# maxrossi91/moni-align

Measured on AMD Instinct MI355X. Metric: aligned reads/s (whole node), 150 bp SE, mouse-chr19-scale x12-haplotype index, higher is better.
Workload: dtype u64/int32

## Files before the change

include/moni_hip.h:

```cpp
#ifndef MONI_HIP_H
#define MONI_HIP_H

#include <stddef.h>
#include <stdint.h>

#ifdef __cplusplus
extern "C" {
#endif

#define MONI_OK 0
#define MONI_EINVAL (-22)
#define MONI_ENOMEM (-12)
#define MONI_EIO (-5)
#define MONI_ENODEV (-19)
#define MONI_ERANGE (-34)

typedef struct moni_index moni_index_t;
typedef struct moni_ctx moni_ctx_t;

typedef struct {
    uint64_t n;
    uint64_t r;
    uint64_t w;
    uint64_t n_seq;
// ... 46 lines not shown
    uint32_t n_cigar;
    uint32_t cigar_off;
} moni_dp_result_t;

typedef struct {
    uint64_t q_off, t_off;
    int32_t qlen, tlen;
    int32_t flag;
    int32_t reserved;
} moni_dp_task_t;

typedef struct {
    int8_t m;
    int8_t mat[25];
    int8_t q, e;
    int32_t w, zdrop, end_bonus;
} moni_dp_params_t;

int moni_index_create(const moni_flat_index_t *flat, int device, moni_index_t **out);
int moni_index_load(const char *path, int device, moni_index_t **out);
void moni_index_destroy(moni_index_t *idx);
uint64_t moni_index_n(const moni_index_t *idx);
uint64_t moni_index_r(const moni_index_t *idx);
uint64_t moni_index_device_bytes(const moni_index_t *idx);
int moni_index_text(const moni_index_t *idx, uint8_t *out, uint64_t cap);

int moni_ctx_create(moni_index_t *idx, moni_ctx_t **out);
void moni_ctx_destroy(moni_ctx_t *ctx);
int moni_reads_upload(moni_ctx_t *ctx, const moni_read_batch_t *batch);
int moni_reads_swap(moni_ctx_t *ctx, uint32_t slot);

int moni_ms_run(moni_ctx_t *ctx);
int moni_ms_query_batch(moni_ctx_t *ctx, const moni_read_batch_t *batch, uint64_t *pointers);

int moni_ms_lengths_batch(moni_ctx_t *ctx, const moni_read_batch_t *batch, uint64_t *pointers, uint64_t *lengths);

typedef struct { uint32_t seg_len;
                 uint32_t overlap;
                 uint32_t reserved[2]; } moni_mslong_params_t;
typedef struct { uint64_t patterns, bases, segments, flagged, chain_runs;
                 uint64_t steps_spec, steps_chain, jumps;
                 double t_walk, t_len, t_chain, t_total;
               } moni_mslong_stats_t;
void moni_mslong_params_default(moni_mslong_params_t *p);
int  moni_ms_long_batch(moni_ctx_t *ctx, const moni_read_batch_t *batch, const moni_mslong_params_t *prm,
                        uint64_t *pointers, uint64_t *lengths, moni_mslong_stats_t *stats);

int moni_seed_run(moni_ctx_t *ctx, const moni_seed_params_t *prm);
int moni_seed_counts(moni_ctx_t *ctx, uint64_t *n_mems, uint64_t *n_occs);
int moni_seed_fetch(moni_ctx_t *ctx, moni_mem_t *mems, uint64_t *occs, uint64_t *read_mem_off);
int moni_seed_batch(moni_ctx_t *ctx, const moni_read_batch_t *batch, const moni_seed_params_t *prm,
                    moni_mem_t **mems, uint64_t *n_mems, uint64_t **occs, uint64_t *n_occs, uint64_t **read_mem_off);
void moni_free(void *p);

int moni_phi_lcp_batch(moni_ctx_t *ctx, const uint64_t *pos, uint64_t n, int inverse, uint64_t *out_pos, uint64_t *out_lcp);

int moni_extz_batch(moni_ctx_t *ctx, const moni_dp_params_t *prm, const uint8_t *qseq, uint64_t qseq_len,
                    const uint8_t *tseq, uint64_t tseq_len, const moni_dp_task_t *tasks, uint64_t n_tasks,
                    moni_dp_result_t *results, uint32_t *cigar_pool, uint64_t cigar_pool_cap, uint64_t *cigar_pool_used);

typedef struct {
    uint32_t min_len, ext_len, check_k, region_dist;
    uint32_t filter_seeds, n_seeds_thr, filter_freq, left_mem_check;
    double freq_thr;
    int8_t smatch, smismatch, gapo, gapo2, gape, gape2;
    int32_t end_bonus, w, zdrop;
    int64_t max_dist_x, max_dist_y, max_iter, max_pred, min_chain_score, min_chain_length;
    uint32_t host_threads;
    uint32_t reserved;
} moni_align_params_t;

typedef struct {
    uint64_t reads, aligned, dp_tasks, dp_cells, dp_rounds;
    double t_seed, t_chain, t_dp, t_host;
    double t_dp_kernel;
    uint64_t handed_back;
    uint64_t dp_reused, dp_cells_reused;
    uint64_t kernel_fallback;
    uint64_t dp_ref_bytes;
    double t_k_chain, t_k_dp, t_k_select, t_k_finish;
    uint64_t handover_why[12];
    uint64_t dp_cells_cut;
    uint64_t dp_slots;
} moni_align_stats_t;

void moni_align_params_default(moni_align_params_t *p);
int moni_align_batch(moni_ctx_t *ctx, const moni_read_batch_t *batch, const uint8_t *names, const uint64_t *name_off,
                     const uint8_t *quals, const moni_align_params_t *prm, char **sam, uint64_t *sam_len,
                     moni_align_stats_t *stats);
int moni_align_run(moni_ctx_t *ctx, const uint8_t *names, const uint64_t *name_off, const uint8_t *quals,
                   const moni_align_params_t *prm, char **sam, uint64_t *sam_len, moni_align_stats_t *stats);
int moni_align_stream(moni_ctx_t *ctx, const moni_read_batch_t *batch, const uint8_t *names, const uint64_t *name_off,
                      const uint8_t *quals, const moni_align_params_t *prm, char **sam, uint64_t *sam_len,
                      moni_align_stats_t *stats);
int moni_align_csv_batch(moni_ctx_t *ctx, const moni_read_batch_t *batch, const uint8_t *names, const uint64_t *name_off,
                         const uint8_t *quals, const moni_align_params_t *prm, char **sam, uint64_t *sam_len,
                         char **csv, uint64_t *csv_len, moni_align_stats_t *stats);
int moni_report_mems_batch(moni_ctx_t *ctx, const moni_read_batch_t *batch, const uint8_t *names, const uint64_t *name_off,
                           const uint8_t *quals, const moni_align_params_t *prm, char **sam, uint64_t *sam_len);
typedef struct {
    uint32_t filter_dir, find_orphan;
    double dir_thr;
    uint64_t ins_learning_n;
    uint64_t ins_learning_score_gap_threshold;
    uint32_t secondary_chains, reserved;
} moni_pe_params_t;
typedef struct {
    double mean, std_dev, variance, sample_variance, m2;
    uint64_t count;
    uint32_t complete, reserved;
} moni_pe_model_t;
void moni_pe_params_default(moni_pe_params_t *p);
int moni_pe_learn_batch(moni_ctx_t *ctx, const moni_read_batch_t *batch, const moni_align_params_t *prm,
                        const moni_pe_params_t *pe, moni_pe_model_t *model);
int moni_pe_align_batch(moni_ctx_t *ctx, const moni_read_batch_t *batch, const uint8_t *names, const uint64_t *name_off,
                        const uint8_t *quals, const moni_align_params_t *prm, const moni_pe_params_t *pe,
                        const moni_pe_model_t *model, char **sam, uint64_t *sam_len, moni_align_stats_t *stats);
int moni_pe_align_stream(moni_ctx_t *ctx, const moni_read_batch_t *batch, const uint8_t *names, const uint64_t *name_off,
                        const uint8_t *quals, const moni_align_params_t *prm, const moni_pe_params_t *pe,
                        const moni_pe_model_t *model, char **sam, uint64_t *sam_len, moni_align_stats_t *stats);
int moni_pe_align_run(moni_ctx_t *ctx, const uint8_t *names, const uint64_t *name_off, const uint8_t *quals, const moni_align_params_t *prm,
                      const moni_pe_params_t *pe, const moni_pe_model_t *model, char **sam, uint64_t *sam_len, moni_align_stats_t *stats);
int moni_pe_align_csv_batch(moni_ctx_t *ctx, const moni_read_batch_t *batch, const uint8_t *names, const uint64_t *name_off,
                            const uint8_t *quals, const moni_align_params_t *prm, const moni_pe_params_t *pe,
                            const moni_pe_model_t *model, char **sam, uint64_t *sam_len, char **csv, uint64_t *csv_len,
                            moni_align_stats_t *stats);
int moni_pe_report_mems_batch(moni_ctx_t *ctx, const moni_read_batch_t *batch, const uint8_t *names, const uint64_t *name_off,
                              const uint8_t *quals, const moni_align_params_t *prm, const moni_pe_params_t *pe, char **sam, uint64_t *sam_len);
typedef struct {
    uint32_t min_len, ext_len;
    int8_t smatch, smismatch, gapo, gape;
    int32_t end_bonus, w, zdrop;
    uint32_t reserved;
} moni_extend_params_t;
typedef struct {
    uint64_t reads, extended, records;
    uint64_t dp_tasks, dp_cells;
    double t_kernel;
} moni_extend_stats_t;
void moni_extend_params_default(moni_extend_params_t *p);
int moni_extend_batch(moni_ctx_t *ctx, const moni_read_batch_t *batch, const uint8_t *names, const uint64_t *name_off, const uint8_t *quals,
                      const moni_extend_params_t *prm, char **sam, uint64_t *sam_len, moni_extend_stats_t *stats);
int moni_extend_run(moni_ctx_t *ctx, const uint8_t *names, const uint64_t *name_off, const uint8_t *quals, const moni_extend_params_t *prm,
                    char **sam, uint64_t *sam_len, moni_extend_stats_t *stats);
int moni_sam_header(const moni_index_t *idx, char **sam, uint64_t *sam_len);

int moni_pml_batch(moni_ctx_t *ctx, const moni_read_batch_t *batch, uint32_t thr,
                   uint32_t *lengths, uint32_t *read_max, uint32_t *read_hits);
int moni_pml_run(moni_ctx_t *ctx, uint32_t thr);
int moni_pml_fetch(moni_ctx_t *ctx, uint32_t *lengths, uint32_t *read_max, uint32_t *read_hits);
int moni_pml_sizes(moni_ctx_t *ctx, uint64_t *n_reads, uint64_t *total_len);

#define MONI_SCREEN_BINS 32
#define MONI_SCREEN_PRESENT 1u
#define MONI_SCREEN_STRAND1 2u
#define MONI_SCREEN_SHORT 4u
typedef struct { uint32_t window;
                 uint32_t min_win;
                 uint32_t ks_num, ks_den;
                 uint32_t strands;
                 uint32_t reserved[3]; } moni_screen_params_t;
typedef struct { uint32_t n_win, n_pos[2], d_max[2], max_pml[2], flags; } moni_screen_res_t;
void moni_screen_params_default(moni_screen_params_t *p);
int moni_screen_run(moni_ctx_t *ctx, const moni_screen_params_t *prm);
int moni_screen_sizes(moni_ctx_t *ctx, uint64_t *n_reads);
int moni_screen_fetch(moni_ctx_t *ctx, moni_screen_res_t *res);
// ... 82 lines not shown
```

moni_align_amd/capi.py:

```python
from __future__ import annotations

import ctypes as C
import os
import subprocess
from typing import Dict, Optional

import numpy as np

os.environ.setdefault("GPU_MAX_HW_QUEUES", "16")

HERE = os.path.dirname(os.path.abspath(__file__))
CSRC = os.path.join(HERE, "csrc")
LIB_PATH = os.environ.get("MONI_HIP_LIB") or os.path.join(CSRC, "libmoni_hip.so")

EXPORTS = [
    "moni_version", "moni_index_create", "moni_index_load", "moni_index_destroy", "moni_index_n", "moni_index_r",
    "moni_index_device_bytes", "moni_index_text", "moni_ctx_create", "moni_ctx_destroy", "moni_reads_upload", "moni_reads_swap", "moni_ms_run",
    "moni_ms_query_batch", "moni_seed_run", "moni_seed_counts", "moni_seed_fetch", "moni_seed_batch", "moni_free",
    "moni_phi_lcp_batch", "moni_extz_batch", "moni_last_kernel_ms", "moni_last_counters", "moni_seed_occ_stats",
    "moni_seed_prefilter", "moni_seed_prefilter_stats",
    "moni_align_params_default", "moni_align_batch", "moni_align_csv_batch", "moni_align_run", "moni_align_stream", "moni_sam_header",
    "moni_ldx_info", "moni_ldx_rewrite", "moni_ldx_lift_batch", "moni_ldx_write",
    "moni_ms_file_info", "moni_ms_file_read", "moni_ms_file_write", "moni_index_load_reference", "moni_ms_lengths_batch", "moni_report_mems_batch",
    "moni_pe_params_default", "moni_pe_learn_batch", "moni_pe_align_batch", "moni_pe_align_stream", "moni_pe_align_run", "moni_pe_align_csv_batch", "moni_pe_report_mems_batch",
    "moni_extend_params_default", "moni_extend_batch", "moni_extend_run",
    "moni_pml_batch", "moni_pml_run", "moni_pml_fetch", "moni_pml_sizes",
    "moni_screen_params_default", "moni_screen_run", "moni_screen_sizes", "moni_screen_fetch", "moni_screen_batch",
    "moni_locate_params_default", "moni_locate_run", "moni_locate_sizes", "moni_locate_fetch", "moni_locate_batch",
    "moni_seqcount_params_default", "moni_seqcount_run", "moni_seqcount_sizes", "moni_seqcount_fetch", "moni_seqcount_batch",
    "moni_loci_params_default", "moni_loci_run", "moni_loci_sizes", "moni_loci_fetch", "moni_loci_batch",
    "moni_approx_params_default", "moni_approx_run", "moni_approx_sizes", "moni_approx_fetch", "moni_approx_batch",
    "moni_mslong_params_default", "moni_ms_long_batch",
]


class FlatIndexC(C.Structure):
    _fields_ = [("n", C.c_uint64), ("r", C.c_uint64), ("w", C.c_uint64), ("n_seq", C.c_uint64),
                ("F", C.c_void_p), ("heads", C.c_void_p), ("starts", C.c_void_p), ("ssa", C.c_void_p),
                ("esa", C.c_void_p), ("thr", C.c_void_p), ("slcp", C.c_void_p), ("text", C.c_void_p),
                ("seq_starts", C.c_void_p), ("seq_names", C.c_char_p),
                ("lift_second", C.c_void_p), ("lift_len", C.c_void_p), ("lift_ins_off", C.c_void_p), ("lift_ins", C.c_void_p),
                ("lift_del_off", C.c_void_p), ("lift_del", C.c_void_p)]


class ReadBatchC(C.Structure):
    _fields_ = [("seq", C.c_void_p), ("offsets", C.c_void_p), ("n_reads", C.c_uint64)]


class SeedParamsC(C.Structure):
    _fields_ = [("min_len", C.c_uint32), ("filter_seeds", C.c_uint32), ("n_seeds_thr", C.c_uint32),
                ("report_mems", C.c_uint32)]


class AlignParamsC(C.Structure):
    _fields_ = [("min_len", C.c_uint32), ("ext_len", C.c_uint32), ("check_k", C.c_uint32), ("region_dist", C.c_uint32),
                ("filter_seeds", C.c_uint32), ("n_seeds_thr", C.c_uint32), ("filter_freq", C.c_uint32), ("left_mem_check", C.c_uint32),
                ("freq_thr", C.c_double),
                ("smatch", C.c_int8), ("smismatch", C.c_int8), ("gapo", C.c_int8), ("gapo2", C.c_int8), ("gape", C.c_int8), ("gape2", C.c_int8),
                ("end_bonus", C.c_int32), ("w", C.c_int32), ("zdrop", C.c_int32),
                ("max_dist_x", C.c_int64), ("max_dist_y", C.c_int64), ("max_iter", C.c_int64), ("max_pred", C.c_int64),
                ("min_chain_score", C.c_int64), ("min_chain_length", C.c_int64),
                ("host_threads", C.c_uint32), ("reserved", C.c_uint32)]


class AlignStatsC(C.Structure):
    _fields_ = [("reads", C.c_uint64), ("aligned", C.c_uint64), ("dp_tasks", C.c_uint64), ("dp_cells", C.c_uint64), ("dp_rounds", C.c_uint64),
                ("t_seed", C.c_double), ("t_chain", C.c_double), ("t_dp", C.c_double), ("t_host", C.c_double),
                ("t_dp_kernel", C.c_double), ("handed_back", C.c_uint64), ("dp_reused", C.c_uint64), ("dp_cells_reused", C.c_uint64),
                ("kernel_fallback", C.c_uint64), ("dp_ref_bytes", C.c_uint64),
                ("t_k_chain", C.c_double), ("t_k_dp", C.c_double), ("t_k_select", C.c_double), ("t_k_finish", C.c_double),
                ("handover_why", C.c_uint64 * 12), ("dp_cells_cut", C.c_uint64), ("dp_slots", C.c_uint64)]


class PeParamsC(C.Structure):
    _fields_ = [("filter_dir", C.c_uint32), ("find_orphan", C.c_uint32), ("dir_thr", C.c_double), ("ins_learning_n", C.c_uint64),
                ("ins_learning_score_gap_threshold", C.c_uint64), ("secondary_chains", C.c_uint32), ("reserved", C.c_uint32)]


class PeModelC(C.Structure):
    _fields_ = [("mean", C.c_double), ("std_dev", C.c_double), ("variance", C.c_double), ("sample_variance", C.c_double), ("m2", C.c_double),
                ("count", C.c_uint64), ("complete", C.c_uint32), ("reserved", C.c_uint32)]


class ExtendParamsC(C.Structure):
    _fields_ = [("min_len", C.c_uint32), ("ext_len", C.c_uint32),
                ("smatch", C.c_int8), ("smismatch", C.c_int8), ("gapo", C.c_int8), ("gape", C.c_int8),
                ("end_bonus", C.c_int32), ("w", C.c_int32), ("zdrop", C.c_int32), ("reserved", C.c_uint32)]


class ExtendStatsC(C.Structure):
    _fields_ = [("reads", C.c_uint64), ("extended", C.c_uint64), ("records", C.c_uint64), ("dp_tasks", C.c_uint64), ("dp_cells", C.c_uint64),
                ("t_kernel", C.c_double)]


class ScreenParamsC(C.Structure):
    _fields_ = [("window", C.c_uint32), ("min_win", C.c_uint32), ("ks_num", C.c_uint32), ("ks_den", C.c_uint32), ("strands", C.c_uint32),
                ("reserved", C.c_uint32 * 3)]


class LocateParamsC(C.Structure):
    _fields_ = [("strands", C.c_uint32), ("max_occ", C.c_uint32), ("reserved", C.c_uint32 * 2)]


class SeqcountParamsC(C.Structure):
    _fields_ = [("strands", C.c_uint32), ("reserved", C.c_uint32), ("max_walk", C.c_uint64)]


class LociParamsC(C.Structure):
    _fields_ = [("strands", C.c_uint32), ("lift", C.c_uint32), ("max_walk", C.c_uint64), ("max_total", C.c_uint64), ("reserved", C.c_uint64 * 2)]


class ApproxParamsC(C.Structure):
    _fields_ = [("strands", C.c_uint32), ("k", C.c_uint32), ("max_hits", C.c_uint32), ("max_occ", C.c_uint32), ("chunk_len", C.c_uint32), ("reserved", C.c_uint32),
                ("max_steps", C.c_uint64)]


class MslongParamsC(C.Structure):
    _fields_ = [("seg_len", C.c_uint32), ("overlap", C.c_uint32), ("reserved", C.c_uint32 * 2)]


class MslongStatsC(C.Structure):
    _fields_ = [("patterns", C.c_uint64), ("bases", C.c_uint64), ("segments", C.c_uint64), ("flagged", C.c_uint64), ("chain_runs", C.c_uint64),
                ("steps_spec", C.c_uint64), ("steps_chain", C.c_uint64), ("jumps", C.c_uint64),
                ("t_walk", C.c_double), ("t_len", C.c_double), ("t_chain", C.c_double), ("t_total", C.c_double)]


class DpParamsC(C.Structure):
    _fields_ = [("m", C.c_int8), ("mat", C.c_int8 * 25), ("q", C.c_int8), ("e", C.c_int8),
                ("w", C.c_int32), ("zdrop", C.c_int32), ("end_bonus", C.c_int32)]


MEM_DTYPE = np.dtype([("pos", "<u8"), ("len", "<u4"), ("idx", "<u4"), ("rpos", "<u4"), ("mate", "<u4"),
                      ("total_occ", "<u4"), ("num_filtered", "<u4"), ("occ_off", "<u8"), ("occ_cnt", "<u4"),
                      ("read", "<u4")])
DP_TASK_DTYPE = np.dtype([("q_off", "<u8"), ("t_off", "<u8"), ("qlen", "<i4"), ("tlen", "<i4"), ("flag", "<i4"),
                          ("reserved", "<i4")])
DP_RESULT_DTYPE = np.dtype([("max", "<i4"), ("max_q", "<i4"), ("max_t", "<i4"), ("mqe", "<i4"), ("mqe_t", "<i4"),
                            ("mte", "<i4"), ("mte_q", "<i4"), ("score", "<i4"), ("reach_end", "<i4"),
                            ("zdropped", "<i4"), ("n_cigar", "<u4"), ("cigar_off", "<u4")])
LOCATE_RES_DTYPE = np.dtype([("count", "<u8"), ("sa_lo", "<u8"), ("occ_off", "<u8"), ("n_occ", "<u4"), ("matched", "<u4")])
SEQCOUNT_RES_DTYPE = np.dtype([("count", "<u8"), ("sa_lo", "<u8"), ("matched", "<u4"), ("n_seqs", "<u4"), ("walked", "<u4"), ("n_segs", "<u4")])
LOCI_RES_DTYPE = np.dtype([("count", "<u8"), ("sa_lo", "<u8"), ("loci_off", "<u8"), ("n_loci", "<u8"), ("matched", "<u4"), ("walked", "<u4"), ("n_segs", "<u4"),
                           ("reserved", "<u4")])
APPROX_RES_DTYPE = np.dtype([("cnt", "<u8", (4,)), ("n_hits", "<u8"), ("hit_off", "<u8"), ("n_kept", "<u4"), ("complete", "<u4"), ("matched", "<u4"), ("reserved", "<u4")])
APPROX_HIT_DTYPE = np.dtype([("task", "<u8"), ("n_mis", "<u4"), ("n_occ", "<u4"), ("sa_lo", "<u8"), ("count", "<u8"), ("occ_off", "<u8")])
APPROX_MAX_STEPS_DEFAULT = 1 << 20
APPROX_CHUNK_LEN_DEFAULT = 1 << 30
assert LOCATE_RES_DTYPE.itemsize == 32 and SEQCOUNT_RES_DTYPE.itemsize == 32 and APPROX_RES_DTYPE.itemsize == 64 and APPROX_HIT_DTYPE.itemsize == 40
assert LOCI_RES_DTYPE.itemsize == 48
SCREEN_RES_DTYPE = np.dtype([("n_win", "<u4"), ("n_pos", "<u4", (2,)), ("d_max", "<u4", (2,)), ("max_pml", "<u4", (2,)), ("flags", "<u4")])
SCREEN_BINS, SCREEN_PRESENT, SCREEN_STRAND1, SCREEN_SHORT = 32, 1, 2, 4
assert SCREEN_RES_DTYPE.itemsize == 32 and C.sizeof(ScreenParamsC) == 32
assert MEM_DTYPE.itemsize == 48 and DP_TASK_DTYPE.itemsize == 32 and DP_RESULT_DTYPE.itemsize == 48

# ... 789 lines not shown
```

moni_align_amd/csrc/align_fast.hip:

```cpp
#pragma once
#include <hip/hip_runtime.h>
#include <stdint.h>

#include "align_core.h"
#include "chain_core.h"
#include "render_core.h"

#define AF_MAX_MEMS 64
#define AF_MAX_ANCH 256
#define AF_MAX_CHAINS 128
#define AF_MAX_CAND 16
#define AF_PLAN_AN 96
#define AF_FIN_AN 16
#define AF_FIN_TB 12
#define AF_MAX_READ 512
#define AF_QCAP 256
#define AF_TB 104
#define AF_BLK 52
#define AF_LPASS (AF_TB / AF_BLK)
#define AF_TS 32
#define AF_GBLK 104
#define AF_GPASS 3
#define AF_NBIN 99
#define AF_BIN_SMALL 16u
#define AF_NSMALL 3u
#define AF_BIN_BAND 19u
#define AF_BIN_GLOBAL 35u
#define AF_BIN_GBAND 51u
#define AF_BIN_WILD 67u
#define AF_BIN_GWILD 83u
#define AF_BANDW 16
#define AF_BIN_PROV ((uint32_t)AF_NBIN)
#define AF_POS_BITS 25
static_assert(AF_NBIN + 1 <= (1 << (32 - AF_POS_BITS)), "task_pos");
#define AF_TB_CIG 24
#define AF_FIN_CIG 96
#define AF_FIN_LCIG 160
#define AF_TXT_SHARDS 32
#define AF_NEG_INF (-0x40000000)

enum { AF_GAP_NONE = 0, AF_GAP_INS, AF_GAP_DEL0, AF_GAP_TASK, AF_GAP_1X1 };
enum { AF_ST_UNALIGNED = 0, AF_ST_CAND = 1, AF_ST_FALLBACK = 2, AF_ST_FINAL = 3, AF_ST_CHAINS = 4  };

struct af_anchor_t {
    uint64_t occ;
    uint16_t len, idx;
    int16_t gap_val;
    uint8_t gap_kind, pad;
};
__device__ __forceinline__ int32_t af_ins_score(const ac_params_t& P, uint64_t l) {
    const uint64_t c1 = (uint64_t)(int64_t)P.gapo + l * (uint64_t)(int64_t)P.gape, c2 = (uint64_t)(int64_t)P.gapo2 + l * (uint64_t)(int64_t)P.gape2;
    return (int32_t)(0 - (c1 < c2 ? c1 : c2));
}
struct af_cand_t {
    int32_t chain_score;
    uint16_t chain_idx;
    uint8_t n_an, strand;
    uint32_t task0;
    uint8_t has_lc, has_rc, n_gap_tasks, overlap;
    int32_t score;
    uint32_t gtask;
    uint16_t an0, pad;
    uint32_t pad2;
};
static_assert(sizeof(af_cand_t) == 32, "af_cand_t");
#define AF_PLAN_HEADER \
    uint8_t status, n_cand; uint16_t n_chains; \
    int32_t min_score; \
    uint8_t final_cand, n_alt; uint16_t pad;       \
    int32_t score2; \
    uint64_t ref_pos, ref_len;    \
    uint32_t tb0, pad2;
struct af_plan_t {
    AF_PLAN_HEADER
    af_cand_t cand[AF_MAX_CAND];
    af_anchor_t an[AF_PLAN_AN];
    uint64_t alt_pos[AF_MAX_CAND];
    int32_t alt_score[AF_MAX_CAND];
};
static_assert(offsetof(af_plan_t, cand) == 40, "af_plan_t header");
template <int NC, int NA, int NT>
struct af_plan_lds_t {
    AF_PLAN_HEADER
    af_cand_t cand[NC];
    af_anchor_t an[NA];
    moni_dp_task_t tasks[NT];
    uint32_t n_an;
};
struct af_ctab_t { int32_t score; uint16_t an0; uint8_t cnt, strand; uint64_t left_ref; };
static_assert(sizeof(af_ctab_t) == 16, "af_ctab_t");
#define AF_CTAB 48
struct af_res_t { int32_t mqe, mqe_t, score, flags; };
struct af_chunk_t { uint32_t bin, start, n, qhi; uint64_t dir_off; };
struct af_tb_t { uint32_t n_ops; uint32_t ops[AF_TB_CIG]; };

struct pe_sel_t;
struct af_args_t {
    ak_args_t A;
    uint32_t pe;
    pe_sel_t* pe_sel;
    af_plan_t* plans;
    moni_dp_task_t* tasks; uint32_t task_cap;
    uint8_t* ntasks;
    af_res_t* res;
    uint32_t* bin_q; uint32_t bin_cap;
    uint32_t* task_pos;
    af_chunk_t* chunks; uint32_t chunk_cap;
    uint8_t* dirs; uint64_t dirs_cap;
    uint32_t* tb_task; af_tb_t* tb; uint32_t tb_cap;
    uint32_t* fb_list; uint32_t* fb_n;
    const uint64_t* pat; const moni_u64x2* blk;
    const uint64_t* text2; const uint32_t* exc; uint32_t exc_sh;
    const uint8_t* pflag;
    af_ctab_t* ctab;
    uint32_t* list0; uint32_t* big_list; uint32_t* huge_list;
    unsigned long long* txt_cur;
    uint64_t txt_shard_words;
    uint8_t* fin_scratch; uint64_t fin_stride;
    uint64_t* bnd;
    uint32_t* ctr;
    unsigned long long* prof;
    unsigned long long* prep_prof;
    uint32_t l0_mm, l0_ma;
    uint32_t wave_max;
    uint32_t dbg;
    uint32_t chain_narrow;
};
#ifdef AF_PROFILE
#define AF_STAMP(var) const long long var = clock64()
#define AF_PROF(G, slot, t0, t1) do { if (threadIdx.x == 0 && (G).prof) atomicAdd(&(G).prof[slot], (unsigned long long)((t1) - (t0))); } while (0)
#define AF_ACC(acc, t0, t1) (acc) += (t1) - (t0)
#else
#define AF_STAMP(var) do {} while (0)
#define AF_PROF(G, slot, t0, t1) do {} while (0)
#define AF_ACC(acc, t0, t1) do {} while (0)
#endif
#define AFPP_WAVE 8u
#define AFPP_READ 2u
enum { AFC_TASKS = 0, AFC_FALLBACK = 1, AFC_TRACED = 2, AFC_READ_CUR = 3, AFC_DIRS_OVF = 4, AFC_CELLS = 6 , AFC_DIROFF = 8 ,
       AFC_NCHUNKS = 10 , AFC_CURSOR = 18 , AFC_BIG = 26, AFC_BIG_CUR = 27, AFC_HUGE = 28, AFC_HUGE_CUR = 29, AFC_L0 = 30 ,
       AFC_NT = 31 , AFC_WHY = 32 , AFC_RBYTES = 44 ,
       AFC_QBYTES = 46 ,
       AFC_SLOTS = 48 ,
       AFC_CUTCELLS = 50 ,
       AFC_BANDH = 52 ,
       AFC_BINS = 68 , AFC_WMODE = 172 , AF_NCTR = 192 };
static_assert(AFC_BINS + AF_NBIN + 1 <= AFC_WMODE && AFC_WMODE + 7 <= AF_NCTR && AFC_WHY + 12 <= AFC_RBYTES && AFC_BANDH + 14 <= AFC_BINS && AFC_NCHUNKS + 7 <= AFC_CURSOR && AFC_CURSOR + 7 <= AFC_BIG, "counter layout");
enum { AF_GRP_LARGE = 0, AF_GRP_SMALL = 1, AF_GRP_BAND = 2, AF_GRP_WILD = 3, AF_GRP_GLOBAL = 4, AF_GRP_GBAND = 5, AF_GRP_GWILD = 6 };

struct af_mem_t { uint64_t occ_off; uint32_t nocc; uint16_t len, idx, rpos; uint8_t mate, pad; };
struct af_chain_t { int32_t score; uint16_t off, cnt; uint32_t mate; };
struct af_start_t { int32_t f, j; };
struct af_left_t { uint64_t ref; int64_t score; };
#define AF_MAX_TASKS_READ 64
template <int MA_, int MC_, int MM_, int NC_, int NA_, int NT_, int PE_ = 0, int SEC_ = 0>
struct af_wave_tt {
    static constexpr int MA = MA_, MC = MC_, MM = MM_, NC = NC_, NA = NA_, NT = NT_;
    static constexpr bool SEC = SEC_ != 0;
    static_assert(MC_ <= MA_, "the sorts of the chain starts and of the chains use per-anchor arrays as scratch");
    static constexpr int NSTACK = MA_ <= 128 ? 16 : MA_ <= 512 ? 20 : 24;
    af_mem_t mem[MM_];
    uint64_t anch[MA_];
    af_chain_t chains[MC_];
    uint16_t pool[(MA_ + MC_) * (SEC_ ? 2 : 1)];
    uint32_t n_chains_sh, status_sh, n_tasks;
    union {
        struct {
            lsort::frame stack[NSTACK];
            int32_t f[MA_], msc[MA_];
            int16_t p[MA_], t[MA_];
            af_start_t starts[MC_];
            uint16_t run_start[MA_ + 1];
            uint16_t s_off[MC_], s_cnt[MC_];
            int32_t f2[SEC_ ? MA_ : 1], msc2[SEC_ ? MA_ : 1];
            int16_t p2[SEC_ ? MA_ : 1], t2[SEC_ ? MA_ : 1];
        };
        struct {
            af_plan_lds_t<NC_, NA_, NT_> plan;
            uint64_t left_ref[MC_];
            uint64_t left_ref2[PE_ ? MC_ : 1];
            uint16_t left_idx[MC_];
            int64_t diff[8];
        };
    };
};
static_assert(AF_MAX_TASKS_READ <= 255, "ntasks is a byte");
typedef af_wave_tt<96, 48, 24, 8, 32, 32> af_wave_small_t;
typedef af_wave_tt<192, 96, 32, 16, 64, 48> af_wave_mid_t;
typedef af_wave_tt<AF_MAX_ANCH, AF_MAX_CHAINS, AF_MAX_MEMS, AF_MAX_CAND, AF_PLAN_AN, AF_MAX_TASKS_READ> af_wave_t;
typedef af_wave_tt<2048, 1024, 256, AF_MAX_CAND, AF_PLAN_AN, AF_MAX_TASKS_READ> af_wave_huge_t;

enum { AF_WHY_LONG = 0, AF_WHY_ANCHORS, AF_WHY_CHAINS, AF_WHY_CANDS, AF_WHY_CHAIN_LEN, AF_WHY_TASK_SIZE, AF_WHY_OVERLAP, AF_WHY_WILDCARD, AF_WHY_LOOP, AF_WHY_REACH_END,
       AF_WHY_CAPACITY, AF_WHY_CIGAR, AF_WHY_N };
#define AF_FALLBACK(G, why) (atomicAdd(&(G).ctr[AFC_WHY + (why)], 1u), (uint32_t)AF_ST_FALLBACK)
#define AF_X(a) ((a) & MONI_POS_MASK_)
#define MONI_POS_MASK_ ((1ull << 40) - 1)

__device__ __forceinline__ uint32_t af_large_bin(int q) {
    if (q <= 16) return q <= 8 ? 0u : q <= 13 ? 1u : 2u;
    if (q <= 32) return 3u + (uint32_t)((q - 17) >> 3);
    if (q <= 160) return 5u + (uint32_t)((q - 33) >> 4);
    return 13u + (uint32_t)((q - 161) >> 5);
}
__device__ __forceinline__ uint32_t af_large_qhi(uint32_t b) { return b < 3 ? (b == 0 ? 8u : b == 1 ? 13u : 16u) : b < 5 ? 24u + 8u * (b - 3) : b < 13 ? 48u + 16u * (b - 5) : 192u + 32u * (b - 13); }
static_assert(AF_QCAP == 256, "af_large_bin covers query lengths up to 256");
__device__ __forceinline__ uint32_t af_bin_of(int qlen, int tlen) {
    return (qlen <= AF_TS && tlen <= AF_TS) ? AF_BIN_SMALL + (qlen <= 8 ? 0u : qlen <= 16 ? 1u : 2u) : af_large_bin(qlen);
}
__device__ __forceinline__ uint32_t af_grp_of_bin(uint32_t bin) {
    return bin < AF_BIN_SMALL ? AF_GRP_LARGE : bin < AF_BIN_BAND ? AF_GRP_SMALL : bin < AF_BIN_GLOBAL ? AF_GRP_BAND : bin < AF_BIN_GBAND ? AF_GRP_GLOBAL : bin < AF_BIN_WILD ? AF_GRP_GBAND
         : bin < AF_BIN_GWILD ? AF_GRP_WILD : AF_GRP_GWILD;
}
__device__ __forceinline__ uint32_t af_grp_b0(uint32_t grp) {
    return grp == AF_GRP_LARGE ? 0u : grp == AF_GRP_SMALL ? AF_BIN_SMALL : grp == AF_GRP_BAND ? AF_BIN_BAND : grp == AF_GRP_GLOBAL ? AF_BIN_GLOBAL : grp == AF_GRP_GBAND ? AF_BIN_GBAND
         : grp == AF_GRP_WILD ? AF_BIN_WILD : AF_BIN_GWILD;
}
__device__ __forceinline__ uint32_t af_grp_b1(uint32_t grp) {
    return grp == AF_GRP_LARGE ? AF_BIN_SMALL : grp == AF_GRP_SMALL ? AF_BIN_BAND : grp == AF_GRP_BAND ? AF_BIN_GLOBAL : grp == AF_GRP_GLOBAL ? AF_BIN_GBAND : grp == AF_GRP_GBAND ? AF_BIN_WILD
         : grp == AF_GRP_WILD ? AF_BIN_GWILD : (uint32_t)AF_NBIN;
}
__device__ __forceinline__ uint32_t af_bin_qhi(uint32_t bin) {
    return bin < AF_BIN_SMALL ? af_large_qhi(bin) : bin < AF_BIN_BAND ? (8u << (bin - AF_BIN_SMALL)) : bin < AF_BIN_GLOBAL ? af_large_qhi(bin - AF_BIN_BAND)
         : bin < AF_BIN_GBAND ? (bin - AF_BIN_GLOBAL + 1u) * 16u : bin < AF_BIN_WILD ? af_large_qhi(bin - AF_BIN_GBAND) : bin < AF_BIN_GWILD ? af_large_qhi(bin - AF_BIN_WILD)
         : (bin - AF_BIN_GWILD + 1u) * 16u;
}
__device__ __forceinline__ uint32_t af_grp_tb(uint32_t grp) {
    return grp == AF_GRP_SMALL ? AF_TS : (grp == AF_GRP_GLOBAL || grp == AF_GRP_GWILD) ? AF_GBLK : (grp == AF_GRP_BAND || grp == AF_GRP_GBAND) ? AF_BANDW : AF_BLK;
}
// ... 95 lines not shown
                const uint32_t iK = K < nA ? (uint32_t)ipos[K] : 0xFFFFFFFFu, jK1 = K > 0 ? (uint32_t)jpos[K - 1] : 0xFFFFFFFFu;
                const long cut = (long)g.uni(iK < jK1 ? iK : jK1);
#pragma unroll
                for (int c = 0; c < NC; ++c) {
                    if (fa[c] && ra[c] < K) a[jpos[ra[c]]] = v[c];
                    if (fb[c] && rb[c] < K) a[ipos[rb[c]]] = v[c];
                }
                __syncthreads();
                if (lane == 0) st[sp] = lsort::frame{(int)cut, (int)last, (int)depth};
                ++sp;
                last = cut;
                __syncthreads();
            }
            for (uint32_t i = (uint32_t)first + (uint32_t)lane; i < (uint32_t)last; i += GW) piece[i] = (uint32_t)first | ((uint32_t)last << 16);
        }
    } else {
        for (uint32_t i = (uint32_t)lane; i < n; i += GW) piece[i] = n << 16;
    }
    __syncthreads();
    T v[NC]; uint32_t rk[NC];
#pragma unroll
    for (int c = 0; c < NC; ++c) {
        const uint32_t i = (uint32_t)lane + GW * c;
        rk[c] = 0;
        if (i < n) {
            v[c] = a[i];
            const auto kx = key(v[c]);
            const uint32_t pc = piece[i], p0 = pc & 0xFFFFu, p1 = pc >> 16;
            rk[c] = p0;
            for (uint32_t k = p0; k < p1; ++k) { const auto kk = key(a[k]); rk[c] += (kk < kx || (kk == kx && k < i)) ? 1u : 0u; }
        }
    }
    __syncthreads();
#pragma unroll
    for (int c = 0; c < NC; ++c) if ((uint32_t)lane + GW * c < n) a[rk[c]] = v[c];
    __syncthreads();
}

template <class I, class U, class WT>
__device__ __forceinline__ void af_chain_run(WT& L, const ac_params_t& P, uint32_t fb, uint32_t fe, float avg_mem_length, const bool sec) {
    const I max_iter = (I)P.max_iter, max_dist_y = (I)P.max_dist_y;
    const U max_pred = (U)P.max_pred;
    const long long max_dist_x = P.max_dist_x;
    I lb = (I)fb;
    for (uint32_t i = fb; i < fe; ++i) {
        const uint64_t aw = L.anch[i];
        const af_mem_t mi = L.mem[aw >> 40];
        const long long x_i = (long long)AF_X(aw);
        const I y_i = mi.rpos, w_i = mi.len;
        const uint32_t mate_i = mi.mate;
        I max_f = w_i, max_j = -1, max_sec_f = w_i, max_sec_j = -1;
        U n_pred = 0;
        if ((U)i - (U)lb > (U)max_iter) lb = (I)i - max_iter;
        for (I j = (I)i - 1; j >= lb; --j) {
            const uint64_t awj = L.anch[j];
            const af_mem_t mj = L.mem[awj >> 40];
            const long long x_j = (long long)AF_X(awj);
            const I y_j = mj.rpos;
            const uint32_t mate_j = mj.mate;
            if (mate_i != mate_j && ((mate_i ^ mate_j) != 3)) continue;
            if (x_i > x_j + max_dist_x) { lb = j; continue; }
            I gain;
            if (!cc_gain<I>((I)(x_i - x_j), y_i, y_j, w_i, mate_i == mate_j, max_dist_y, avg_mem_length, gain)) continue;
            const I score = (I)L.f[j] + gain;
            if (score > max_f) { max_f = score; max_j = j; if (n_pred > 0) --n_pred; }
            else if (WT::SEC && sec && (I)L.f2[j] + gain > max_sec_f) {
                if (max_j >= 0) {
                    const uint64_t pos_j = (uint64_t)x_j - mj.len + 1;
                    bool uniq = true;
                    for (I tmp = max_j; tmp >= 0; tmp = L.p[tmp]) { const uint64_t at = L.anch[tmp]; if (AF_X(at) - L.mem[at >> 40].len + 1 == pos_j) { uniq = false; break; } }
                    if (uniq) { max_sec_f = (I)L.f2[j] + gain; max_sec_j = j; }
                }
            }
            else if ((U)(I)L.t[j] == (U)i && (++n_pred > max_pred)) break;
            if (L.p[j] > 0) L.t[L.p[j]] = (int16_t)i;
            if (WT::SEC && sec && L.p2[j] > 0) L.t2[L.p2[j]] = (int16_t)i;
        }
        L.f[i] = (int32_t)max_f; L.p[i] = (int16_t)max_j;
        L.msc[i] = (max_j >= 0 && L.msc[max_j] > max_f) ? L.msc[max_j] : (int32_t)max_f;
        if (WT::SEC && sec) { L.f2[i] = (int32_t)max_sec_f; L.p2[i] = (int16_t)max_sec_j; L.msc2[i] = (max_sec_j >= 0 && L.msc2[max_sec_j] > max_sec_f) ? L.msc2[max_sec_j] : (int32_t)max_sec_f; }
    }
}

template <class WT, class GT = af_grp_t<64>, bool GEN = true>
__device__ __forceinline__ uint32_t af_chain(const af_args_t& G, WT& L, uint32_t na, float avg_mem_length, const GT g = GT(), const bool sec_on = false) {
    const ac_params_t& P = G.A.P;
    constexpr uint32_t GW = GT::W;
    const int lane = g.lane;
    na = g.uni(na);
    AF_STAMP(s0);
#if defined(AF_PROFILE) || defined(AF_CUTS)
    if (G.dbg & 32) {  } else
#endif
    if (GEN && (G.dbg & 64)) {
        if (na <= 16) af_small_sort(L.anch, na, [](const uint64_t& a, const uint64_t& b) { return AF_X(a) < AF_X(b); }, lane);
        else { if (lane == 0) lsort::sort(L.anch, (long)na, [](const uint64_t& a, const uint64_t& b) { return AF_X(a) < AF_X(b); }, L.stack); __syncthreads(); }
    } else {
        af_wave_sort<(WT::MA + GT::W - 1) / GT::W>(g, L.anch, na, L.stack, L.run_start, reinterpret_cast<uint16_t*>(L.p), reinterpret_cast<uint32_t*>(L.f), [](const uint64_t& x) { return AF_X(x); });
        for (uint32_t i = lane; i < na; i += GW) L.p[i] = 0;
        __syncthreads();
    }
    AF_STAMP(s1); AF_PROF(G, 5, s0, s1);
    uint32_t n_runs = 0;
    for (uint32_t i0 = 0; i0 < na; i0 += GW) {
        const uint32_t i = i0 + lane;
        const bool brk = i < na && (i == 0 || (long long)AF_X(L.anch[i]) > (long long)AF_X(L.anch[i - 1]) + P.max_dist_x);
        const unsigned long long bal = g.ballot(brk);
        if (brk) L.run_start[n_runs + (uint32_t)__popcll(bal & ((1ull << lane) - 1ull))] = (uint16_t)i;
        n_runs += (uint32_t)__popcll(bal);
    }
    if (lane == 0) L.run_start[n_runs] = (uint16_t)na;
    __syncthreads();
#if defined(AF_PROFILE) || defined(AF_CUTS)
    if (G.dbg & 128) return AF_ST_UNALIGNED;
#endif
    for (uint32_t k = lane; k < n_runs; k += GW) {
        const uint32_t fb = L.run_start[k], fe = L.run_start[k + 1];
        if (!GEN || (G.chain_narrow && !(G.dbg & 64))) af_chain_run<int32_t, uint32_t>(L, P, fb, fe, avg_mem_length, WT::SEC && sec_on);
        else af_chain_run<long long, size_t>(L, P, fb, fe, avg_mem_length, WT::SEC && sec_on);
    }
    __syncthreads();
    AF_STAMP(s2); AF_PROF(G, 6, s1, s2);
#if defined(AF_PROFILE) || defined(AF_CUTS)
    if (G.dbg & 256) return AF_ST_UNALIGNED;
#endif
    uint32_t n_chains = 0;
    auto track = [&](int32_t* F, int32_t* MSC, int16_t* PP, int16_t* TT, uint32_t pool0, bool by_score_alone, uint32_t& n_starts) -> bool {
        for (uint32_t i = lane; i < na; i += GW) TT[i] = 0;
        __syncthreads();
        for (uint32_t i = lane; i < na; i += GW) if (PP[i] >= 0) TT[PP[i]] = 1;
        __syncthreads();
        uint32_t ns = 0;
        for (uint32_t i0 = 0; i0 < na; i0 += GW) {
            const uint32_t i = i0 + lane;
            const bool is_end = i < na && TT[i] == 0 && MSC[i] > P.min_chain_score;
            af_start_t st; st.f = 0; st.j = 0;
            if (is_end) { uint32_t j = i; while (F[j] < MSC[j]) j = (uint32_t)PP[j]; st.f = F[j]; st.j = (int32_t)j; }
            const unsigned long long bal = g.ballot(is_end);
            const uint32_t at = ns + (uint32_t)__popcll(bal & ((1ull << lane) - 1ull));
            if (is_end && at < (uint32_t)WT::MC) L.starts[at] = st;
            ns += (uint32_t)__popcll(bal);
        }
        n_starts = ns;
        if (ns > (uint32_t)WT::MC) return false;
        __syncthreads();
        if (ns == 0) return true;
        if (by_score_alone) {
            af_wave_sort<(WT::MC + GT::W - 1) / GT::W>(g, L.starts, ns, L.stack, reinterpret_cast<uint16_t*>(TT), L.s_off, reinterpret_cast<uint32_t*>(L.pool + pool0), [](const af_start_t& x) { return -(int64_t)x.f; });
        } else {
            af_start_t v[(WT::MC + GT::W - 1) / GT::W]; uint32_t rk[(WT::MC + GT::W - 1) / GT::W];
#pragma unroll
            for (int q = 0; q < (WT::MC + GT::W - 1) / GT::W; ++q) {
                const uint32_t s = (uint32_t)lane + GW * q;
                rk[q] = 0;
                if (s < ns) { v[q] = L.starts[s]; for (uint32_t k = 0; k < ns; ++k) { const af_start_t w = L.starts[k]; rk[q] += (w.f > v[q].f || (w.f == v[q].f && (w.j > v[q].j || (w.j == v[q].j && k < s)))) ? 1u : 0u; } }
            }
            __syncthreads();
#pragma unroll
            for (int q = 0; q < (WT::MC + GT::W - 1) / GT::W; ++q) if ((uint32_t)lane + GW * q < ns) L.starts[rk[q]] = v[q];
            __syncthreads();
        }
        for (uint32_t i = lane; i < na; i += GW) TT[i] = 0;
        __syncthreads();
        for (uint32_t k = lane; k < n_runs; k += GW) {
            const uint32_t fb = L.run_start[k], fe = L.run_start[k + 1];
            uint32_t used = pool0 + fb;
            for (uint32_t s = 0; s < ns; ++s) used += (uint32_t)L.starts[s].j < fb ? 1u : 0u;
            uint32_t s = 0;
            while (true) {
                while (s < ns && ((uint32_t)L.starts[s].j < fb || (uint32_t)L.starts[s].j >= fe)) ++s;
                if (s >= ns) break;
                const af_start_t st = L.starts[s];
                long long j = st.j;
                uint32_t cnt = 0;
                const uint32_t off = used;
                const uint32_t mate0 = L.mem[L.anch[j] >> 40].mate;
                uint32_t paired = 0;
                do { paired |= L.mem[L.anch[j] >> 40].mate != mate0 ? 1u : 0u; L.pool[used++] = (uint16_t)j; cnt++; TT[j] = 1; j = PP[j]; } while (j >= 0 && TT[j] == 0);
                bool keep = false;
                if (j < 0) keep = (long long)cnt >= P.min_chain_length;
                else if ((long long)st.f - F[j] >= P.min_chain_score) keep = (long long)cnt >= P.min_chain_length;
                L.s_off[s] = (uint16_t)off; L.s_cnt[s] = (uint16_t)(keep ? (cnt | (paired << 15)) : 0u);
                ++s;
            }
        }
        __syncthreads();
        uint32_t kept = 0;
        for (uint32_t s0 = 0; s0 < ns; s0 += GW) {
            const uint32_t sx = s0 + lane;
            const bool keep = sx < ns && L.s_cnt[sx] > 0;
            const unsigned long long bal = g.ballot(keep);
            const uint32_t at = n_chains + kept + (uint32_t)__popcll(bal & ((1ull << lane) - 1ull));
            if (keep && at < (uint32_t)WT::MC) {
                af_chain_t c;
                c.score = L.starts[sx].f; c.mate = L.mem[L.anch[L.starts[sx].j] >> 40].mate | ((uint32_t)(L.s_cnt[sx] >> 15) << 8); c.off = L.s_off[sx]; c.cnt = L.s_cnt[sx] & 0x7FFFu;
// ... 194 lines not shown
    __syncthreads();
    uint32_t status = L.status_sh;
    if (status != AF_ST_CAND) return status;
    const uint32_t n_cand = PL.n_cand;
    uint32_t nt = 0;
    if ((uint32_t)lane < n_cand) { af_cand_anchors(L, PL.cand[lane], 3u, 0u); nt = af_build_cand<false>(G, L, PL.cand[lane], off, m, 0u); }
    const bool bad = g.ballot(nt == 0xFFFFFFFFu) != 0ull;
    if (bad) { if (lane == 0) L.status_sh = AF_FALLBACK(G, AF_WHY_TASK_SIZE); __syncthreads(); return L.status_sh; }
    uint32_t incl = nt;
    for (int o = 1; o < AF_MAX_CAND; o <<= 1) { const uint32_t x = (uint32_t)__shfl_up((int)incl, o); if (lane >= o) incl += x; }
    const uint32_t total = (uint32_t)g.shfl((int)incl, (int)(n_cand ? n_cand - 1 : 0));
    if (n_cand && total > (uint32_t)WT::NT) {
        if (has_larger) return 0xFFu;
        if (lane == 0) L.status_sh = AF_FALLBACK(G, AF_WHY_CAPACITY);
        __syncthreads();
        return L.status_sh;
    }
    if ((uint32_t)lane < n_cand) {
        PL.cand[lane].task0 = incl - nt;
        af_build_cand<true>(G, L, PL.cand[lane], off, m, incl - nt);
    }
    if (lane == 0) L.n_tasks = n_cand ? total : 0u;
    __syncthreads();
    return AF_ST_CAND;
}

__global__ void __launch_bounds__(256) classify_kernel(const af_args_t G) {
    const ak_args_t& A = G.A;
    const uint64_t r_in = (uint64_t)blockIdx.x * 256 + threadIdx.x;
    const int lane = threadIdx.x & 63;
    const unsigned long long lt_mask = lane ? (~0ull >> (64 - lane)) : 0ull;
    uint32_t level = 4;
    uint32_t m = 0;
    if (r_in < A.n_reads) {
        const uint64_t r = A.read_lo + r_in;
        m = (uint32_t)(A.offs[r + 1] - A.offs[r]);
        const uint64_t a = A.read_mem_off[r], b = A.read_mem_off[r + 1];
        if (m >= AF_MAX_READ || (b - a) > (uint64_t)af_wave_huge_t::MM) level = 3;
        else {
            unsigned long long total = 0;
            for (uint64_t k = a; k < b; ++k) total += A.mems[k].occ_cnt;
            uint32_t n_mems = 0; unsigned long long n_anch = 0;
            for (uint64_t k = a; k < b; ++k) {
                const uint32_t oc = A.mems[k].occ_cnt;
                bool keep = true;
                if (A.P.filter_freq) { const double fr = static_cast<double>(oc) / (double)(size_t)total; if (fr > A.P.freq_thr) keep = false; }
                if (keep) { ++n_mems; n_anch += oc; }
            }
            level = (n_mems <= G.l0_mm && n_anch <= (unsigned long long)G.l0_ma) ? 0u
                  : (n_mems <= (uint32_t)af_wave_t::MM && n_anch <= (unsigned long long)af_wave_t::MA) ? 1u
                  : (n_mems <= (uint32_t)af_wave_huge_t::MM && n_anch <= (unsigned long long)af_wave_huge_t::MA) ? 2u : 3u;
        }
    }
#pragma unroll
    for (uint32_t lv = 0; lv < 3; ++lv) {
        const unsigned long long bal = __ballot(level == lv);
        if (!bal) continue;
        uint32_t base = 0;
        const int lead = __ffsll((long long)bal) - 1;
        if (lane == lead) base = atomicAdd(&G.ctr[lv == 0 ? AFC_L0 : lv == 1 ? AFC_BIG : AFC_HUGE], (uint32_t)__popcll(bal));
        base = (uint32_t)__shfl((int)base, lead);
        if (level == lv) (lv == 0 ? G.list0 : lv == 1 ? G.big_list : G.huge_list)[base + (uint32_t)__popcll(bal & lt_mask)] = (uint32_t)r_in;
    }
    if (level == 3) {
        af_plan_t& PL = G.plans[r_in];
        PL.status = AF_ST_FALLBACK; PL.n_cand = 0; PL.n_chains = 0; PL.final_cand = 0; PL.n_alt = 0; PL.pad = 0; PL.score2 = 0; PL.ref_pos = PL.ref_len = 0; PL.tb0 = 0; PL.pad2 = 0;
        PL.min_score = A.min_score_of_len[m <= A.max_len ? m : A.max_len];
        G.ntasks[r_in] = 0;
        G.fb_list[atomicAdd(G.fb_n, 1u)] = (uint32_t)(A.read_lo + r_in);
        atomicAdd(&G.ctr[AFC_WHY + (m >= AF_MAX_READ ? AF_WHY_LONG : AF_WHY_ANCHORS)], 1u);
    }
}

template <class WT, int LEVEL, bool GEN, class GT>
__device__ __forceinline__ void af_plan_read(const af_args_t& G, WT& L, const GT g, uint32_t r_in, uint64_t off, uint32_t m, uint32_t na, float avg, bool fallback, bool too_big) {
    constexpr uint32_t GW = GT::W;
    const int lane = g.lane;
    const ak_args_t& A = G.A;
    const uint64_t r = A.read_lo + r_in;
    uint32_t status = AF_ST_UNALIGNED;
#if defined(AF_PROFILE) || defined(AF_CUTS)
    if (G.dbg & 4) na = 0;
#endif
    if (!fallback && !too_big && na > 0) {
        status = af_chain<WT, GT, GEN>(G, L, na, avg, g);
        status = (uint32_t)g.shfl((int)status, 0);
        __syncthreads();
#if defined(AF_PROFILE) || defined(AF_CUTS)
        if ((G.dbg & 8) && status == AF_ST_CAND) status = AF_ST_UNALIGNED;
#endif
        if (status == 0xFFu) too_big = true;
        else if (status == AF_ST_CAND) {
            for (uint32_t ci = lane; ci < L.n_chains_sh; ci += GW) {
                const af_chain_t ch = L.chains[ci];
                const uint64_t aw = L.anch[L.pool[ch.off + ch.cnt - 1]];
                const af_mem_t ml = L.mem[aw >> 40];
                L.left_ref[ci] = ac_seq_off(A.P, ac_lift(A.P, AF_X(aw) - ml.len + 1)) + 1;
            }
            __syncthreads();
#if defined(AF_PROFILE) || defined(AF_CUTS)
            if (G.dbg & 16) status = AF_ST_UNALIGNED; else
#endif
            if (LEVEL == 0 && (uint32_t)WT::MC <= AF_CTAB && (uint32_t)WT::MA <= AF_PLAN_AN && G.ctab != nullptr) {
                const uint32_t n_chains = L.n_chains_sh;
                af_ctab_t* const CT = G.ctab + (size_t)r_in * AF_CTAB;
                af_anchor_t* const AN = G.plans[r_in].an;
                uint32_t an0 = 0;
                for (uint32_t c0 = 0; c0 < n_chains; c0 += GW) {
                    const uint32_t ci = c0 + (uint32_t)lane;
                    const uint32_t cnt = ci < n_chains ? L.chains[ci].cnt : 0u;
                    uint32_t incl = cnt;
                    for (int o = 1; o < (int)GW; o <<= 1) { const uint32_t x = (uint32_t)__shfl_up((int)incl, o); if (lane >= o) incl += x; }
                    if (ci < n_chains) {
                        const af_chain_t ch = L.chains[ci];
                        const uint32_t at = an0 + incl - cnt;
                        uint32_t strand = 0;
                        for (uint32_t k = 0; k < ch.cnt; ++k) {
                            const uint64_t aw = L.anch[L.pool[ch.off + ch.cnt - 1 - k]];
                            const af_mem_t mk = L.mem[aw >> 40];
                            af_anchor_t X; X.occ = AF_X(aw) - mk.len + 1; X.len = mk.len; X.idx = mk.idx; X.gap_val = 0; X.gap_kind = AF_GAP_NONE; X.pad = 0;
                            AN[at + k] = X;
                            if (k == 0) strand = (mk.mate & 2) ? 1u : 0u;
                        }
                        af_ctab_t E; E.score = ch.score; E.an0 = (uint16_t)at; E.cnt = (uint8_t)ch.cnt; E.strand = (uint8_t)strand; E.left_ref = L.left_ref[ci];
                        CT[ci] = E;
                    }
                    an0 += (uint32_t)g.shfl((int)incl, (int)GW - 1);
                }
                if (lane == 0) {
                    af_plan_t& PH = G.plans[r_in];
                    PH.status = AF_ST_CHAINS; PH.n_cand = 0; PH.n_chains = (uint16_t)n_chains; PH.final_cand = 0; PH.n_alt = 0; PH.pad = 0; PH.score2 = 0; PH.ref_pos = PH.ref_len = 0; PH.tb0 = 0; PH.pad2 = 0;
                    PH.min_score = A.min_score_of_len[m <= A.max_len ? m : A.max_len];
                    G.ntasks[r_in] = 0;
                }
                __syncthreads();
                return;
            }
            status = af_plan_cands(G, L, off, m, g);
            __syncthreads();
            if (status == 0xFFu) too_big = true;
        }
    }
    __syncthreads();
    if (too_big) {
        if (LEVEL == 0) { if (lane == 0) G.big_list[atomicAdd(&G.ctr[AFC_BIG], 1u)] = r_in; return; }
        if (LEVEL == 1) { if (lane == 0) G.huge_list[atomicAdd(&G.ctr[AFC_HUGE], 1u)] = r_in; return; }
        fallback = true;
    }
    if (fallback) { status = AF_ST_FALLBACK; if (lane == 0) atomicAdd(&G.ctr[AFC_WHY + (m >= AF_MAX_READ ? AF_WHY_LONG : AF_WHY_ANCHORS)], 1u); }
    auto& PL = L.plan;
    const uint32_t nt = status == AF_ST_CAND ? L.n_tasks : 0u;
    const uint32_t t0 = r_in * AF_MAX_TASKS_READ;
    if (status == AF_ST_CAND) {
        for (uint32_t k = lane; k < nt; k += GW) G.tasks[t0 + k] = PL.tasks[k];
        if ((uint32_t)lane < PL.n_cand) PL.cand[lane].task0 += t0;
    }
    if (lane == 0) G.ntasks[r_in] = (uint8_t)nt;
    if (lane == 0) {
        if (status != AF_ST_CAND) { PL.n_cand = 0; PL.n_chains = 0; }
        PL.status = (uint8_t)status; PL.final_cand = 0; PL.n_alt = 0; PL.pad = 0; PL.score2 = 0; PL.ref_pos = PL.ref_len = 0; PL.tb0 = 0; PL.pad2 = 0;
        PL.min_score = A.min_score_of_len[m <= A.max_len ? m : A.max_len];
        if (status == AF_ST_FALLBACK) G.fb_list[atomicAdd(G.fb_n, 1u)] = (uint32_t)r;
    }
    __syncthreads();
    {
        const uint32_t words = (uint32_t)((offsetof(af_plan_t, cand) + (status == AF_ST_CAND ? PL.n_cand : 0u) * sizeof(af_cand_t)) / 4);
        const uint32_t* src = reinterpret_cast<const uint32_t*>(&PL);
        uint32_t* dst = reinterpret_cast<uint32_t*>(G.plans + r_in);
        for (uint32_t w = lane; w < words; w += GW) dst[w] = src[w];
        const uint32_t awords = status == AF_ST_CAND ? PL.n_an * (uint32_t)(sizeof(af_anchor_t) / 4) : 0u;
        const uint32_t* asrc = reinterpret_cast<const uint32_t*>(PL.an);
        uint32_t* adst = reinterpret_cast<uint32_t*>(G.plans[r_in].an);
        for (uint32_t w = lane; w < awords; w += GW) adst[w] = asrc[w];
    }
    __syncthreads();
}

template <class WT, int LEVEL, int OCC = (LEVEL == 0 ? 6 : LEVEL == 1 ? 3 : 1), int GW = 64, bool GEN = false>
__global__ void __launch_bounds__(64) __attribute__((amdgpu_waves_per_eu(OCC, OCC))) chain_plan_kernel(const af_args_t G) {
    constexpr uint32_t NG = 64 / GW;
    __shared__ WT Ls[NG];
    typedef af_grp_t<GW> GT;
    const GT g;
    WT& L = Ls[NG > 1 ? g.id() : 0];
    const int lane = g.lane;
    const ak_args_t& A = G.A;
    constexpr bool BIG = LEVEL > 0;
    const uint32_t n_work = G.ctr[LEVEL == 0 ? AFC_L0 : LEVEL == 1 ? AFC_BIG : AFC_HUGE];
    const uint32_t* const work_list = LEVEL == 0 ? G.list0 : LEVEL == 1 ? G.big_list : G.huge_list;
    constexpr uint32_t GRAB = BIG ? 1u : NG > 1 ? 2u : 8u;
    uint32_t w_base = 0, w_k = GRAB;
    while (true) {
        if (w_k >= GRAB) {
            if (threadIdx.x == 0) w_base = atomicAdd(&G.ctr[LEVEL == 0 ? AFC_READ_CUR : LEVEL == 1 ? AFC_BIG_CUR : AFC_HUGE_CUR], GRAB * NG);
            w_base = GW == 64 ? (uint32_t)__builtin_amdgcn_readfirstlane((int)w_base) : (uint32_t)__shfl((int)w_base, 0);
            w_k = 0;
        }
        if (w_base + w_k * NG >= n_work) break;
        const uint32_t w_in = w_base + w_k * NG + (NG > 1 ? (uint32_t)g.id() : 0u);
        ++w_k;
        if (w_in >= n_work) continue;
        const uint32_t r_in = g.uni(work_list[w_in]);
        const uint64_t r = A.read_lo + r_in;
        const uint64_t off = A.offs[r];
        const uint32_t m = (uint32_t)(A.offs[r + 1] - off);
        const uint64_t a = A.read_mem_off[r], b = A.read_mem_off[r + 1];
        if (lane == 0) L.n_tasks = 0;
        bool fallback = m >= AF_MAX_READ || (b - a) > 4 * AF_MAX_MEMS;
        bool too_big = false;
        uint32_t n_mems = 0, na = 0;
        float avg = 0.f;
        if (!fallback && b > a) {
            unsigned long long total = 0;
            for (uint64_t k = a + lane; k < b; k += GW) total += A.mems[k].occ_cnt;
            for (int o = GW / 2; o > 0; o >>= 1) total += __shfl_xor(total, o);
            unsigned long long tot_len = 0, n_anch = 0;
            for (uint64_t k0 = a; k0 < b; k0 += GW) {
                const uint64_t k = k0 + lane;
                bool keep = false;
                moni_mem_t gm;
                if (k < b) {
                    gm = A.mems[k];
                    keep = true;
                    if (A.P.filter_freq) { const double fr = static_cast<double>(gm.occ_cnt) / (double)(size_t)total; if (fr > A.P.freq_thr) keep = false; }
                }
                const unsigned long long bal = g.ballot(keep);
                const uint32_t at = n_mems + (uint32_t)__popcll(bal & g.lt_mask());
                if (keep && at < (uint32_t)WT::MM) {
                    af_mem_t x; x.occ_off = gm.occ_off; x.nocc = gm.occ_cnt; x.len = (uint16_t)gm.len; x.idx = (uint16_t)gm.idx; x.rpos = (uint16_t)gm.rpos; x.mate = (uint8_t)gm.mate; x.pad = 0;
                    L.mem[at] = x;
                }
                if (keep) { tot_len += (unsigned long long)gm.len * gm.occ_cnt; n_anch += gm.occ_cnt; }
                n_mems += (uint32_t)__popcll(bal);
            }
            for (int o = GW / 2; o > 0; o >>= 1) { tot_len += __shfl_xor(tot_len, o); n_anch += __shfl_xor(n_anch, o); }
            if (n_mems > (uint32_t)WT::MM || n_anch > (unsigned long long)WT::MA) too_big = true;
            na = g.uni((uint32_t)n_anch);
            if (!too_big && na > 0) {
                avg = (float)(size_t)tot_len / (size_t)n_anch;
                __syncthreads();
                for (uint32_t x = lane; x < na; x += GW) {
                    uint32_t i = 0, base = 0;
                    while (base + L.mem[i].nocc <= x) { base += L.mem[i].nocc; ++i; }
                    const af_mem_t mi = L.mem[i];
                    L.anch[x] = (A.occs[mi.occ_off + (x - base)] + mi.len - 1) | ((uint64_t)i << 40);
                }
                for (uint32_t i = lane; i < na; i += GW) { L.f[i] = 0; L.msc[i] = 0; L.p[i] = 0; L.t[i] = 0; }
            }
        }
        __syncthreads();
        af_plan_read<WT, LEVEL, GEN>(G, L, g, r_in, off, m, na, avg, fallback, too_big);
    }
}

struct af_plan_view_t { af_anchor_t* an; moni_dp_task_t* tasks; };
struct af_view_t { af_plan_view_t plan; };
__global__ void __launch_bounds__(256) plan_kernel(const af_args_t G) {
    __shared__ int32_t s_diff[8][256];
    __shared__ uint8_t s_left[AF_CTAB][256];
    const int lane = threadIdx.x;
    const ak_args_t& A = G.A;
    const ac_params_t& P = A.P;
    const uint64_t r_in = (uint64_t)blockIdx.x * 256 + threadIdx.x;
    if (r_in >= A.n_reads) return;
    af_plan_t& PL = G.plans[r_in];
    if (PL.status != AF_ST_CHAINS) return;
    const uint64_t r = A.read_lo + r_in;
    const uint64_t off = A.offs[r];
    const uint32_t m = (uint32_t)(A.offs[r + 1] - off);
    const uint32_t n_chains = PL.n_chains;
    const af_ctab_t* const CT = G.ctab + (size_t)r_in * AF_CTAB;
    const uint32_t t0 = (uint32_t)r_in * AF_MAX_TASKS_READ;
    af_view_t V; V.plan.an = PL.an; V.plan.tasks = G.tasks + t0;
    uint32_t status = AF_ST_CAND, why = AF_WHY_N;
    uint32_t n_diff = 0, n_left = 0, n_cand = 0, n_tasks = 0;
    const uint32_t check_k = P.check_k < 8u ? P.check_k : 8u;
    if (P.check_k > 8u) { status = AF_ST_FALLBACK; why = AF_WHY_CAPACITY; }
    for (uint32_t ci = 0; ci < n_chains && n_diff < check_k && status == AF_ST_CAND; ++ci) {
        const af_ctab_t ch = CT[ci];
        { bool f = false; for (uint32_t q = 0; q < n_diff; ++q) f = f || s_diff[q][lane] == ch.score; if (!f) s_diff[n_diff++][lane] = ch.score; }
        if (P.left_mem_check) {
            bool seen = false;
            for (uint32_t k = 0; k < n_left; ++k) {
                const af_ctab_t o = CT[s_left[k][lane]];
                const uint64_t d = o.left_ref > ch.left_ref ? o.left_ref - ch.left_ref : ch.left_ref - o.left_ref;
                if (d < P.region_dist && o.score == ch.score) seen = true;
            }
            if (seen) continue;
            s_left[n_left][lane] = (uint8_t)ci; ++n_left;
        }
        if (n_diff >= check_k) continue;
        if (n_cand >= AF_MAX_CAND) { status = AF_ST_FALLBACK; why = AF_WHY_CANDS; break; }
        af_cand_t C;
        C.chain_score = ch.score; C.chain_idx = (uint16_t)ci; C.n_an = ch.cnt; C.task0 = t0 + n_tasks; C.has_lc = C.has_rc = C.n_gap_tasks = 0; C.overlap = 0; C.score = 0; C.gtask = 0;
        C.strand = ch.strand; C.an0 = ch.an0; C.pad = 0; C.pad2 = 0;
        if (n_tasks + 1u + ch.cnt > AF_MAX_TASKS_READ) { status = AF_ST_FALLBACK; why = AF_WHY_CAPACITY; break; }
        const uint32_t nt = af_build_cand<2>(G, V, C, off, m, n_tasks);
        if (nt == 0xFFFFFFFFu) { status = AF_ST_FALLBACK; why = AF_WHY_TASK_SIZE; break; }
        n_tasks += nt;
        PL.cand[n_cand++] = C;
    }
    if (status == AF_ST_FALLBACK) {
        atomicAdd(&G.ctr[AFC_WHY + why], 1u);
        G.fb_list[atomicAdd(G.fb_n, 1u)] = (uint32_t)r;
        PL.status = AF_ST_FALLBACK; PL.n_cand = 0; PL.n_chains = 0;
        G.ntasks[r_in] = 0;
        return;
    }
    PL.status = AF_ST_CAND; PL.n_cand = (uint8_t)n_cand;
    G.ntasks[r_in] = (uint8_t)n_tasks;
}

#define AF_BT_READS 32u
#define AF_T_WILDQ 0x4000
__device__ __forceinline__ void af_global_band(const dp_launch_t& D, const moni_dp_task_t& T, int& dmin, int& dmax, bool* saw_wild = nullptr);
__device__ __forceinline__ void af_ext_band(const dp_launch_t& D, const moni_dp_task_t& T, int& dmin, int& dmax);
__global__ void __launch_bounds__(256) bin_tasks_kernel(const af_args_t G) {
    __shared__ uint32_t cnt[AF_NBIN + 1], base[AF_NBIN + 1], ovf[AF_BT_READS];
    static_assert(AF_MAX_TASKS_READ == 64, "bin_tasks_kernel: 4 reads x 64 slots per round");
    constexpr uint32_t ROUNDS = AF_BT_READS / 4;
    const uint32_t tid = threadIdx.x;
    const uint64_t n_reads = G.A.n_reads;
    if (blockIdx.x == 0 && tid == 0) G.ctr[AFC_TASKS] = (uint32_t)n_reads * AF_MAX_TASKS_READ;
    if (tid <= AF_NBIN) cnt[tid] = 0;
    if (tid < AF_BT_READS) ovf[tid] = 0;
    __syncthreads();
    const uint32_t k = tid & 63u;
    uint32_t bin[ROUNDS], local[ROUNDS];
    bool valid[ROUNDS];
#pragma unroll
    for (uint32_t q = 0; q < ROUNDS; ++q) {
        const uint64_t r_in = (uint64_t)blockIdx.x * AF_BT_READS + 4 * q + (tid >> 6);
        valid[q] = r_in < n_reads && k < (uint32_t)G.ntasks[r_in];
        bin[q] = 0; local[q] = 0;
        if (valid[q]) {
// ... 1939 lines not shown
                    const bool on = k0 + lane < n_lcig;
                    uint32_t it = l_it, len = l_len, in2 = l_inc;
                    if (k0) { it = on ? S[AFP_LCIG + k0 + lane] : 0u; len = on ? afr_cig_len(it) : 0u; in2 = afr_wave_scan(len); }
                    if (on) afr_put_cig(L.line + b + in2 - len, it, lit);
                    b += afr_lane(in2, 63);
                }
                const uint64_t lifted = (uint64_t)afr_lane(hw, AFP_H_LIFTED_LO) | ((uint64_t)afr_lane(hw, AFP_H_LIFTED_HI) << 32);
                auto base_at = [&](uint32_t o) { const uint64_t ta = lifted + o; return dp_nt4(ta < A.D.n_text ? A.D.text[ta] : 0u); };
                b = md_at;
                for (uint32_t k0 = 0; k0 < n_md; k0 += 64) {
                    const bool on = k0 + lane < n_md;
                    uint32_t it = d_it, len = d_len, in2 = d_inc;
                    if (k0) { it = on ? S[AFP_MD + k0 + lane] : 0u; len = on ? afr_md_len(it) : 0u; in2 = afr_wave_scan(len); }
                    if (on) afr_put_md(L.line + b + in2 - len, it, lit, base_at);
                    b += afr_lane(in2, 63);
                }
                if (strand) { _Pragma("unroll 2") for (uint32_t k = lane; k < m; k += 64) L.line[s_at + k] = ak_compl(A.D.reads[off + m - 1 - k]); }
                else { _Pragma("unroll 2") for (uint32_t k = lane; k < m; k += 64) L.line[s_at + k] = A.D.reads[off + k]; }
                if (has_q) { _Pragma("unroll 2") for (uint32_t k = lane; k < m; k += 64) L.line[q_at + k] = F.quals[strand ? off + m - 1 - k : off + k]; }
            }
        }
        if (!to_host) {
            if (!afr_fits(p)) { to_host = true; if (lane == 0) atomicAdd(&G.ctr[AFC_WHY + AF_WHY_CAPACITY], 1u); }
            else { _Pragma("unroll 1") for (uint32_t k = lane; k < rn; k += 64) L.line[k] = (uint8_t)F.rnames[n0 + k]; }
        }
        __syncthreads();
        if (to_host) rec.status = 2;
        else {
            const unsigned long long words = (unsigned long long)((p + 7) >> 3);
            const uint32_t shard = blockIdx.x % AF_TXT_SHARDS;
            unsigned long long to = 0;
            if (lane == 0) to = atomicAdd(&G.txt_cur[shard * 8], words);
            to = ((unsigned long long)(uint32_t)__shfl((int)(to >> 32), 0) << 32) | (uint32_t)__shfl((int)(to & 0xFFFFFFFFull), 0);
            if (to + words > G.txt_shard_words) rec.status = 2;
            else {
                to += (unsigned long long)(shard + 1) * G.txt_shard_words;
                const uint64_t* src = reinterpret_cast<const uint64_t*>(L.line);
                for (unsigned long long k = lane; k < words; k += 64) F.txt_pool[to + k] = src[k];
                rec.txt_len = p; rec.txt_off = to;
            }
        }
        if (lane == 0) {
            A.recs[r_in] = rec;
            if (A.dev_len) {
                A.dev_len[r_in] = rec.txt_len; A.dev_off[r_in] = rec.txt_off;
                if (rec.status == 2 || rec.txt_len == 0) atomicAdd(&A.dev_sum[0], 1ull);
                else if (rec.status == 1) atomicAdd(&A.dev_sum[8 + 8 * (blockIdx.x % 16)], 1ull);
            }
        }
    }
}

__global__ void __launch_bounds__(256) gather_lines_kernel(const uint64_t* __restrict__ pool, const uint64_t* __restrict__ len, const uint64_t* __restrict__ off,
                                                           const uint64_t* __restrict__ pos, uint64_t n_reads, uint8_t* __restrict__ out) {
    const int lane = threadIdx.x & 63;
    const uint64_t wave = ((uint64_t)blockIdx.x * 256 + threadIdx.x) >> 6, n_waves = ((uint64_t)gridDim.x * 256) >> 6;
    for (uint64_t r = wave; r < n_reads; r += n_waves) {
        const uint64_t l = len[r];
        const uint8_t* __restrict__ src = reinterpret_cast<const uint8_t*>(pool + off[r]);
        uint8_t* __restrict__ dst = out + pos[r];
        const uint64_t head = l < 8 ? l : ((8 - (reinterpret_cast<uintptr_t>(dst) & 7)) & 7);
        if ((uint64_t)lane < head) dst[lane] = src[lane];
        const uint64_t words = (l - head) >> 3;
        for (uint64_t k = lane; k < words; k += 64) {
            uint64_t w;
            memcpy(&w, src + head + 8 * k, 8);
            *reinterpret_cast<uint64_t*>(dst + head + 8 * k) = w;
        }
        const uint64_t done = head + 8 * words;
        if (done + lane < l) dst[done + lane] = src[done + lane];
    }
}
__global__ void gather_summary_kernel(const uint64_t* __restrict__ len, const uint64_t* __restrict__ pos, uint64_t n_reads, const unsigned long long* __restrict__ dev_sum,
                                      unsigned long long* __restrict__ out3) {
    if (threadIdx.x == 0 && blockIdx.x == 0) {
        out3[0] = n_reads ? pos[n_reads - 1] + len[n_reads - 1] : 0ull;
        out3[1] = dev_sum[0];
        unsigned long long al = dev_sum[1];
        for (int s = 0; s < 16; ++s) al += dev_sum[8 + 8 * s];
        out3[2] = al;
    }
}

static inline uint32_t af_wave_max() { const char* v = getenv("MONI_AF_WAVE_MAX"); return v ? (uint32_t)strtoul(v, nullptr, 10) : 96u; }
static inline void af_launch_dp(const af_args_t& G, hipStream_t sx, unsigned dp_grid, unsigned n_cu, uint64_t n_units) {
    if (!(G.dbg & 0x20000u)) hipLaunchKernelGGL(band_tasks_kernel, dim3((unsigned)((G.bin_cap + 255) / 256)), dim3(256), 0, sx, G);
    hipLaunchKernelGGL(af_chunk_kernel, dim3(1), dim3(64), 0, sx, G, (uint32_t)AF_GRP_LARGE, (uint32_t)AF_GRP_WILD);
    hipLaunchKernelGGL((dp_lane_kernel<AF_BLK, AF_QCAP, AF_LPASS>), dim3(dp_grid), dim3(64), 0, sx, G, (uint32_t)AF_GRP_LARGE);
    hipLaunchKernelGGL((dp_lane_kernel<AF_TS, AF_TS, 1>), dim3(dp_grid), dim3(64), 0, sx, G, (uint32_t)AF_GRP_SMALL);
    hipLaunchKernelGGL((dp_band_kernel<AF_BANDW>), dim3(n_cu * 8), dim3(64), 0, sx, G, (uint32_t)AF_GRP_BAND);
    hipLaunchKernelGGL((dp_lane_kernel<AF_BLK, AF_QCAP, AF_LPASS, true>), dim3(dp_grid), dim3(64), 0, sx, G, (uint32_t)AF_GRP_WILD);
    hipLaunchKernelGGL((dp_wave_kernel<AF_BLK, AF_LPASS, 4>), dim3(n_cu * 8), dim3(64), 0, sx, G, (uint32_t)AF_GRP_WILD, (uint32_t)AF_GRP_WILD);
    hipLaunchKernelGGL(global_task_kernel, dim3((unsigned)((n_units + 255) / 256)), dim3(256), 0, sx, G);
    const uint64_t gmax = G.task_cap > n_units * AF_MAX_TASKS_READ ? G.task_cap - n_units * AF_MAX_TASKS_READ : 0;
    if (gmax) hipLaunchKernelGGL(global_band_kernel, dim3((unsigned)((gmax + 255) / 256)), dim3(256), 0, sx, G);
    hipLaunchKernelGGL(af_chunk_kernel, dim3(1), dim3(64), 0, sx, G, (uint32_t)AF_GRP_GLOBAL, (uint32_t)AF_GRP_GWILD);
    hipLaunchKernelGGL((dp_band_kernel<AF_BANDW>), dim3(n_cu * 8), dim3(64), 0, sx, G, (uint32_t)AF_GRP_GBAND);
    hipLaunchKernelGGL((dp_lane_kernel<AF_GBLK, AF_QCAP, AF_GPASS>), dim3(dp_grid), dim3(64), 0, sx, G, (uint32_t)AF_GRP_GLOBAL);
    hipLaunchKernelGGL((dp_lane_kernel<AF_GBLK, AF_QCAP, AF_GPASS, true>), dim3(dp_grid), dim3(64), 0, sx, G, (uint32_t)AF_GRP_GWILD);
    hipLaunchKernelGGL((dp_wave_kernel<AF_GBLK, AF_GPASS, 8>), dim3(n_cu * 8), dim3(64), 0, sx, G, (uint32_t)AF_GRP_GLOBAL, (uint32_t)AF_GRP_GWILD);
}
```

moni_align_amd/csrc/chain_core.h:

```cpp
#pragma once
#include <stdint.h>

#if defined(__HIPCC__) || defined(__CUDACC__)
#define CC_HD __host__ __device__ __forceinline__
#else
#define CC_HD inline
#endif

#define CC_MAX_READ 512
#define CC_NARROW_MAX_DIST (1ll << 28)
#define CC_NARROW_MAX_COUNT (1ll << 30)

CC_HD uint32_t cc_ilog2(uint32_t v) {
#if defined(__HIP_DEVICE_COMPILE__)
    return (uint32_t)(31 - __clz((int)v));
#else
    return (uint32_t)(31 - __builtin_clz(v));
#endif
}

template <class P>
inline bool cc_narrow_ok(const P& p) {
    return p.max_dist_x >= 0 && p.max_dist_x <= CC_NARROW_MAX_DIST && p.max_dist_y >= -CC_NARROW_MAX_DIST && p.max_dist_y <= CC_NARROW_MAX_DIST
        && p.max_iter >= 0 && p.max_iter <= CC_NARROW_MAX_COUNT && p.max_pred >= 0 && p.max_pred <= CC_NARROW_MAX_COUNT;
}

template <class I>
CC_HD bool cc_gain(I x_d, I y_i, I y_j, I w_i, bool same_mate, I max_dist_y, float avg_mem_length, I& gain) {
    const I y_d = y_i - y_j;
    const int32_t l = (int32_t)(y_d > x_d ? (y_d - x_d) : (x_d - y_d));
    const uint32_t ilog_l = l > 0 ? cc_ilog2((uint32_t)l) : 0;
    if (same_mate && (y_j >= y_i || y_d > max_dist_y)) return false;
    const I mn = y_d < x_d ? y_d : x_d;
    const I alpha = mn < w_i ? mn : w_i;
    I beta = 0;
    if (!same_mate) {
        if (x_d == 0) ++beta;
        else { const int c_lin = (int)(l * .01 * avg_mem_length); beta = c_lin < (I)ilog_l ? (I)c_lin : (I)ilog_l; }
    } else {
        beta = l > 0 ? ((I)(.01 * l * avg_mem_length) + (I)ilog_l) >> 1 : 0;
    }
    gain = alpha - beta;
    return true;
}
```

moni_align_amd/csrc/moni_hip.hip:

```cpp
#include <hip/hip_runtime.h>
#include <fcntl.h>
#include <sys/mman.h>
#include <sys/stat.h>
#include <unistd.h>
#include <cstring>
#include <atomic>
#include <chrono>
#include <rocprim/device/device_scan.hpp>
#include <rocprim/device/device_radix_sort.hpp>

#include <sched.h>
#include <cstdio>
#include <cstdlib>
#include <cstring>
#include <string>
#include <thread>
#include <algorithm>
#include <vector>

#include "../../include/moni_hip.h"
#include "owned_buf.hpp"
#include "image.hpp"
#include "lift_build.hpp"
#include "ref_index_io.hpp"
// ... 56 lines not shown
    int device = 0;
    moni_consts_t K;
    DBuf<moni_tables_t> d_tables;
    DBuf<moni_row_t> d_rows;
    DBuf<moni_frow_t> d_frows;
    DBuf<uint32_t> d_cr;
    DBuf<moni_rec_t> d_recs;
    DBuf<moni_phi_t> d_phi, d_phi_inv;
    DBuf<uint32_t> d_phi_dir, d_phi_inv_dir;
    DBuf<uint8_t> d_text;
    DBuf<uint64_t> d_text2; DBuf<uint32_t> d_exc; uint32_t exc_sh = 10, exc_words = 0;
    DBuf<uint32_t> d_kmers; uint32_t pf_k = 0; double pf_density = 0; bool pf_on = false; float pf_build_ms = 0; bool compl_acgt = false;
    DBuf<uint64_t> d_seq_starts;
    DBuf<uint32_t> d_name_id;
    DBuf<uint8_t> d_snames; DBuf<uint32_t> d_sname_off;
    DBuf<moni_lift_seq_t> d_lift_seqs; DBuf<moni_lift_run_t> d_lift_runs;
    DBuf<uint64_t> d_pdir;
    bool lifts_null = true;
    uint64_t bytes = 0;
    std::vector<uint8_t> h_text;
    mh::HostIndex hix;
};

#define PE_NSET 1
#define PE_NSTREAM 4
#ifndef AK_NSET
#define AK_NSET 2
#endif
struct ResidentBatch {
    DBuf<uint8_t> seq;
    DBuf<uint64_t> offs;
    uint64_t n_reads = 0, total_len = 0, max_len = 0;
    DBuf<moni_u64x2> blk; std::vector<moni_u64x2> h_blk;
    std::vector<uint8_t> h_seq;
    std::vector<uint64_t> h_offs;
};
struct moni_ctx : ResidentBatch {
    moni_index* idx = nullptr;
    Stream stream;
    Event ev[EV_N];
    bool ev_valid[EV_N] = {};
    std::vector<ResidentBatch> stash;
    DBuf<uint64_t> ptr, pat; DBuf<uint8_t> pflag;
    DBuf<uint32_t> cnt_m, cnt_s;
    DBuf<uint64_t> pf_flag, pf_pos, pf_live; DBuf<unsigned long long> pf_stats;
    int seed_prefilter = 1;
    bool seed_fuse = true;
    DBuf<uint64_t> evl; DBuf<uint32_t> evl_cnt;
    bool ms_events = true;
    bool pf_active = false;
    uint64_t pf_tasks = 0;
    DBuf<moni_u64x2> mem_slots;
    DBuf<uint64_t> tot, read_mem_off;
    DBuf<moni_mem_t> mems;
    DBuf<uint32_t> aux;
    DBuf<uint64_t> lowers, tmp;
    DBuf<uint64_t> long_list;
    DBuf<uint64_t> occ_cnt, occ_off, occs;
    DBuf<moni_mem_t> mems_compact;
    bool occs_valid = false;
    uint64_t ovf_cap = 4096;
    uint64_t occ_stats[6] = {0, 0, 0, 0, 0, 0};
    DBuf<uint32_t> pool;
    DBuf<uint8_t> scan_tmp;
    DBuf<occ_small_t> d_small;
    DBuf<unsigned long long> d_counters;
    uint64_t n_mems = 0, n_occs = 0;
    uint32_t dirs_scale = 1;
    uint32_t tmp_cap = 16;
    uint32_t pool_rows = 4096;
    double dp_kernel_ms_accum = 0;
    int extz_lds = 0;
    int ms_variant = 0;
    DBuf<uint8_t> dp_q, dp_t, dp_dir;
    DBuf<moni_dp_task_t> dp_tasks;
    DBuf<moni_dp_result_t> dp_res;
    DBuf<uint32_t> dp_cig;
    DBuf<uint64_t> dp_off;
    DBuf<uint32_t> dp_ws;
    DBuf<dp_big_t> dp_big;
    DBuf<uint8_t> dp_dir_big;
    struct AfSet {
        DBuf<af_plan_t> plans; DBuf<moni_dp_task_t> tasks; DBuf<af_res_t> res; DBuf<uint32_t> bin_q, task_pos, tb_task, big_list, ctr; DBuf<uint8_t> ntasks;
        DBuf<af_chunk_t> chunks; DBuf<uint8_t> dirs, fin; DBuf<uint32_t> recipes; DBuf<af_ctab_t> ctab; DBuf<af_tb_t> tb; DBuf<uint64_t> bnd; DBuf<unsigned long long> prof, prep_prof, txt_cur;
    } af[AK_NSET], af_pe[PE_NSET];
    HBuf<unsigned long long> pe_hcur;
    HBuf<uint32_t> af_ctr_host;
    DBuf<uint32_t> fb_all;
    DBuf<ak_slot_t> ak_slots;
    DBuf<ak_wave_t> ak_waves;
    DBuf<unsigned long long> ak_cursors;
    bool mapq_tab_ready = false;
    DBuf<uint8_t> ak_rnames, ak_quals; DBuf<uint64_t> ak_rname_off, ak_txt; DBuf<double> ak_mapq_tab;
    HBuf<uint64_t> h_txt;
    uint64_t ak_waves_full = 0;
    Stream ak_stream[AK_NSET], copy_stream, fb_stream[AK_NSET], pe_stream[PE_NSTREAM];
    std::vector<Event> ak_fin;
    std::vector<Event> af_ev;
    std::vector<Event> ak_begin, ak_done;
    HBuf<moni_aln_rec_t> h_recs; HBuf<uint32_t> h_cig; HBuf<moni_alt_t> h_alt; HBuf<uint64_t> h_md;
    std::vector<mh::Aligner::OutBuf> pieces;
    std::vector<std::vector<char>> md_scratch;
    DBuf<moni_aln_rec_t> ak_recs;
    DBuf<uint32_t> ak_cig;
    DBuf<moni_alt_t> ak_alt;
    DBuf<int32_t> ak_minscore;
    struct PeBufs { DBuf<pe_slot_t> slots; DBuf<ak_wave_t> waves; DBuf<pe_rec_t> recs; DBuf<uint32_t> cig; DBuf<moni_alt_t> alt; DBuf<unsigned long long> cur; DBuf<int32_t> minscore;
                    DBuf<pe_sel_t> sel[PE_NSET]; DBuf<uint32_t> fb[PE_NSET];
                    DBuf<uint64_t> txt_pool, block, dev_len, dev_off, dev_pos; DBuf<int32_t> subn_tab; DBuf<double> pen_tab; DBuf<pe_pslot_t> park, k1_slots; DBuf<uint8_t> k1_dirs; DBuf<uint32_t> parked; DBuf<pe_orec_t> orec; uint32_t tag = 0;
                    DBuf<uint8_t> scan_tmp[PE_NSTREAM]; bool subn_ready = false;
    } pe;
    DBuf<unsigned long long> d_ak_cursors;
    HBuf<char> out_buf;
    DBuf<uint64_t> ak_block;
    DBuf<uint64_t> ak_dev_len, ak_dev_off, ak_dev_pos; DBuf<unsigned long long> ak_dev_sum;
    HBuf<unsigned long long> h_sum;
    DBuf<uint8_t> gather_tmp[AK_NSET];
    float ak_kernel_ms = 0;
    struct ExBufs {
        DBuf<uint8_t> seq2, rnames, quals, lines, block, dirs; DBuf<uint64_t> rname_off, dir_off, cig_off, len, off, pos; DBuf<ext_plan_t> plans; DBuf<moni_dp_task_t> tasks;
        DBuf<moni_dp_result_t> res; DBuf<uint32_t> cig; DBuf<int32_t> minscore; DBuf<unsigned long long> cur; HBuf<unsigned long long> hcur;
        DBuf<moni_tables_t> tables;
    } ex;
    struct PmlBufs {
        DBuf<uint32_t> lens, mx, hits; uint64_t n_reads = 0, total = 0; bool valid = false;
    } pml;
    struct ScreenBufs {
        DBuf<moni_screen_res_t> res; uint64_t n_reads = 0; bool valid = false;
    } scr;
    struct LocBufs {
        DBuf<moni_locate_res_t> res; DBuf<uint64_t> toe, cnt, off, pos, seq_off; DBuf<uint32_t> seq; uint64_t n_tasks = 0, n_occ = 0; bool valid = false;
    } loc;
    struct ScBufs {
        DBuf<moni_locate_res_t> lres; DBuf<moni_seqcount_res_t> res; DBuf<uint64_t> toe, cnt, off, counts; DBuf<uint32_t> k_lo;
        uint64_t n_tasks = 0, n_segs = 0; uint32_t n_seq = 0; bool valid = false;
    } sc;
    struct LociBufs {
        DBuf<moni_locate_res_t> lres; DBuf<moni_seqcount_res_t> sres; DBuf<moni_loci_res_t> res; DBuf<uint64_t> toe, cnt, off, occ_off, keys, sorted, idx, lpos, lseq_off, support;
        DBuf<uint32_t> k_lo, lseq; DBuf<uint8_t> sort_tmp;
        uint64_t n_tasks = 0, n_loci = 0, n_segs = 0; bool valid = false;
    } loci;
    struct ApxBufs {
        DBuf<moni_approx_res_t> res; DBuf<moni_approx_hit_t> slots, hits; DBuf<apx_ckpt_t> ckpt; DBuf<uint64_t> cnt, ck_off, hit_off, occ_cnt, occ_off, pos, seq_off; DBuf<uint32_t> seq;
        uint64_t n_tasks = 0, n_hits = 0, n_occ = 0; bool valid = false;
    } apx;
    struct MslBufs {
        DBuf<uint64_t> ptr, cnt, seg_off, head, run_idx; DBuf<uint32_t> lens, flags; DBuf<mslong_seg_t> segs; DBuf<mslong_state_t> states; DBuf<mslong_run_t> runs;
        DBuf<unsigned long long> counters;
    } msl;
    int n_cu_cached = 0, pe_occ_cached = 0;
};

namespace {

template <class Tp>
int upload(DBuf<Tp>& d, const std::vector<Tp>& h, uint64_t& bytes) {
    size_t nb = h.size() * sizeof(Tp);
    if (d.alloc_bytes(nb ? nb : 8)) return MONI_ENOMEM;
    if (nb && hipMemcpy(d.p, h.data(), nb, hipMemcpyHostToDevice) != hipSuccess) return MONI_ENODEV;
    bytes += nb;
    return MONI_OK;
}

int ctx_n_cu(moni_ctx* c) {
    if (!c->n_cu_cached) { hipDeviceProp_t pr; c->n_cu_cached = hipGetDeviceProperties(&pr, c->idx->device) == hipSuccess ? pr.multiProcessorCount : 256; }
    return c->n_cu_cached;
}
// ... 834 lines not shown
                ++li;
                continue;
            }
            std::vector<uint8_t>& S = is_long ? lseq : sseq; std::vector<uint8_t>& N = is_long ? lnm : snm; std::vector<uint8_t>& Q = is_long ? lq : sq;
            std::vector<uint64_t>& O = is_long ? loff : soff; std::vector<uint64_t>& NO = is_long ? lnoff : snoff;
            S.insert(S.end(), b->seq + off, b->seq + off + m); O.push_back(S.size());
            N.insert(N.end(), names + name_off[r], names + name_off[r + 1]); NO.push_back(N.size());
            if (quals) Q.insert(Q.end(), quals + off, quals + off + m);
            if (is_long) ++li;
        }
        char* ssam = nullptr; uint64_t slen = 0;
        moni_align_stats_t st_s; memset(&st_s, 0, sizeof st_s);
        const moni_read_batch_t sb{sseq.data(), soff.data(), (uint64_t)soff.size() - 1};
        int rc = align_core(c, &sb, false, false, snm.data(), snoff.data(), quals ? sq.data() : nullptr, prm, &ssam, &slen, &st_s);
        if (rc) return rc;
        std::string lsam; mh::AlignStats st_l;
        if (loff.size() > 1) {
            const moni_read_batch_t lb{lseq.data(), loff.data(), (uint64_t)loff.size() - 1};
            if ((rc = host_align_subset(c, *prm, lb, lnm.data(), lnoff.data(), quals ? lq.data() : nullptr, lsam, st_l))) { free(ssam); return rc; }
        }
        std::string out;
        out.reserve(slen + lsam.size() + 64 * longs.size());
        size_t ps = 0, pl = 0; li = 0;
        for (uint64_t r = 0; r < NR; ++r) {
            if (li < longs.size() && longs[li] == r) {
                if (!long_line[li].empty()) out += long_line[li];
                else { const size_t e = lsam.find('\n', pl); out.append(lsam, pl, e - pl + 1); pl = e + 1; }
                ++li;
            } else { const char* e = (const char*)memchr(ssam + ps, '\n', slen - ps); const size_t n = (size_t)(e - (ssam + ps)) + 1; out.append(ssam + ps, n); ps += n; }
        }
        free(ssam);
        char* dst = (char*)malloc(out.size() + 1);
        if (!dst) return MONI_ENOMEM;
        memcpy(dst, out.data(), out.size()); dst[out.size()] = 0;
        *sam = dst; *sam_len = out.size();
        if (stats) { *stats = st_s; stats->reads = NR; stats->aligned += st_l.aligned; stats->dp_tasks += st_l.dp_tasks; stats->dp_cells += st_l.dp_cells; stats->handed_back += (uint64_t)loff.size() - 1; }
        return MONI_OK;
    } catch (const std::bad_alloc&) { return MONI_ENOMEM; }
}

int moni_align_stream(moni_ctx_t* c, const moni_read_batch_t* b, const uint8_t* names, const uint64_t* name_off, const uint8_t* quals,
                      const moni_align_params_t* prm, char** sam, uint64_t* sam_len, moni_align_stats_t* stats) {
    if (!c || !b || !prm || !sam || !sam_len || (b->n_reads && (!names || !name_off))) return MONI_EINVAL;
    bool any_long = false;
    for (uint64_t r = 0; r < b->n_reads && !any_long; ++r) any_long = b->offsets[r + 1] - b->offsets[r] >= MONI_LONG_READ;
    if (!any_long) return align_core(c, b, false, true, names, name_off, quals, prm, sam, sam_len, stats);
    char* tmp = nullptr; uint64_t len = 0;
    int rc = moni_align_batch(c, b, names, name_off, quals, prm, &tmp, &len, stats);
    if (rc) return rc;
    HIPCHK(hipSetDevice(c->idx->device));
    if (c->out_buf.ensure_keep(len + 1, 0)) { free(tmp); return MONI_ENOMEM; }
    memcpy(c->out_buf.p, tmp, len); c->out_buf.p[len] = 0;
    free(tmp);
    *sam = c->out_buf.p; *sam_len = len;
    return MONI_OK;
}

int moni_align_run(moni_ctx_t* c, const uint8_t* names, const uint64_t* name_off, const uint8_t* quals, const moni_align_params_t* prm,
                   char** sam, uint64_t* sam_len, moni_align_stats_t* stats) {
    if (!c || !prm || !sam || !sam_len || (c->n_reads && (!names || !name_off))) return MONI_EINVAL;
    if (c->h_offs.size() != c->n_reads + 1) return MONI_EINVAL;
    std::vector<uint8_t> hs = std::move(c->h_seq);
    std::vector<uint64_t> ho = std::move(c->h_offs);
    const moni_read_batch_t view{hs.data(), ho.data(), c->n_reads};
    const uint64_t nr = c->n_reads, tl = c->total_len, ml = c->max_len;
    int rc = align_core(c, &view, true, true, names, name_off, quals, prm, sam, sam_len, stats);
    if (c->n_reads != nr || c->h_offs.size() != 0) {
        const int rc2 = reads_upload(c, &view, false);
        if (!rc) rc = rc2;
    }
    c->h_seq = std::move(hs); c->h_offs = std::move(ho);
    c->n_reads = nr; c->total_len = tl; c->max_len = ml;
    return rc;
}

static int align_core(moni_ctx* c, const moni_read_batch_t* b, bool resident, bool ctx_out, const uint8_t* names, const uint64_t* name_off, const uint8_t* quals,
                      const moni_align_params_t* prm, char** sam, uint64_t* sam_len, moni_align_stats_t* stats) {
    moni_index* I = c->idx;
    HIPCHK(hipSetDevice(I->device));
    c->dp_kernel_ms_accum = 0;
    std::string out;
    mh::AlignStats st;
    uint64_t why_out[12] = {};
    const uint8_t* q = quals ? quals + b->offsets[0] : nullptr;
    static const bool host_only = getenv("MONI_ALIGN_HOST") != nullptr;
    bool out_done = false;
    int rc;
    if (host_only) {
        if ((rc = host_align_subset(c, *prm, *b, names, name_off, q, out, st))) return rc;
    } else {
        if (prm->w >= 0 || prm->zdrop >= 0) return MONI_EINVAL;
        const double t_enter = mh::now_s();
        double t_mark[4] = {0, 0, 0, 0};
        const uint64_t NR = b->n_reads;
        uint64_t sub_min = 250000, sub_mid = 250000;
        if (const char* v = getenv("MONI_ALIGN_SUB")) { const long long x = atoll(v); if (x > 0) sub_min = sub_mid = (uint64_t)x; }
        if (const char* v = getenv("MONI_ALIGN_SUB_MIN")) { const long long x = atoll(v); if (x > 0) sub_min = (uint64_t)x; }
        std::vector<uint64_t> sub_lo(1, 0);
        while (sub_lo.back() < NR) {
            const uint64_t done = sub_lo.back(), rest = NR - done;
            uint64_t take = done == 0 ? sub_min : (rest >= sub_mid + sub_min ? sub_mid : (rest > sub_min + sub_min / 2 ? rest - sub_min : rest));
            if (take > rest) take = rest;
            sub_lo.push_back(done + take);
        }
        const uint64_t n_sub = sub_lo.size() - 1;
        uint64_t sub_reads = 0;
        for (uint64_t k = 0; k < n_sub; ++k) sub_reads = std::max(sub_reads, sub_lo[k + 1] - sub_lo[k]);
        uint64_t force_back = 0;
        if (const char* v = getenv("MONI_AK_FORCE_HANDBACK")) { const long long x = atoll(v); if (x > 0) force_back = (uint64_t)x; }
        if (!c->ak_waves_full) {
            int n_cu = 256, per_cu = 8;
            n_cu = ctx_n_cu(c);
            if (hipOccupancyMaxActiveBlocksPerMultiprocessor(&per_cu, align_kernel, 64, 0) != hipSuccess || per_cu < 1) per_cu = 8;
            c->ak_waves_full = (uint64_t)n_cu * (uint64_t)per_cu;
        }
        const uint64_t waves_full = c->ak_waves_full;
        const int T = prm->host_threads > 0 ? (int)prm->host_threads : 1;
        mh::Pool pool(T);
        mh::Aligner AL(I->hix, *prm, b->seq, b->offsets);
        if ((int)c->pieces.size() < T) c->pieces.resize(T);
        std::vector<std::vector<std::string>> kept(n_sub);
        std::vector<std::vector<uint32_t>> back_of(n_sub);
        std::vector<uint64_t> aligned_t(T, 0);
        double host_busy = 0;
        char* abuf = ctx_out ? c->out_buf.p : nullptr; size_t acap = ctx_out ? c->out_buf.cap : 0, alen = 0; uint64_t eager_upto = 0; bool eager_ok = true, eager_oom = false;
        auto drop_abuf = [&]() { if (!ctx_out) free(abuf); abuf = nullptr; };
        auto grow_abuf = [&](size_t cap) -> bool {
            if (!ctx_out) { char* nb = (char*)realloc(abuf, cap); if (!nb) return false; abuf = nb; acap = cap; return true; }
            if (c->out_buf.ensure_keep(cap, alen)) return false;
            abuf = c->out_buf.p; acap = c->out_buf.cap;
            return true;
        };
        double prof[7] = {0, 0, 0, 0, 0, 0, 0};
        uint64_t why_sum[AF_WHY_N] = {};
        double hist[8] = {0, 0, 0, 0, 0, 0, 0, 0}, cyc[7] = {0, 0, 0, 0, 0, 0, 0};
        uint64_t waves_used = 0;

        const bool gpu_text = getenv("MONI_ALIGN_HOST_FORMAT") == nullptr && NR > 0;
        const bool fin_v1 = getenv("MONI_AF_FIN_V1") != nullptr;
        std::thread uploader;
        int rc_up = MONI_OK;
        if (gpu_text) {
            const uint64_t nb_names = name_off[NR] - name_off[0], nb_q = quals ? b->offsets[NR] - b->offsets[0] : 0;
            if ((rc = c->ak_rnames.ensure(nb_names + 16)) || (rc = c->ak_rname_off.ensure(NR + 1)) || (rc = c->ak_quals.ensure(nb_q + 16))) return rc;
            if (!c->copy_stream) HIPCHK(hipStreamCreateWithFlags(&c->copy_stream.h, hipStreamNonBlocking));
            uploader = std::thread([&, nb_names, nb_q]() {
                if (hipSetDevice(I->device) != hipSuccess) { rc_up = MONI_ENODEV; return; }
                std::vector<uint64_t> rel(NR + 1);
                for (uint64_t r = 0; r <= NR; ++r) rel[r] = name_off[r] - name_off[0];
                if (hipMemcpyAsync(c->ak_rnames.p, names + name_off[0], nb_names, hipMemcpyHostToDevice, c->copy_stream) != hipSuccess ||
                    hipMemcpyAsync(c->ak_rname_off.p, rel.data(), (NR + 1) * 8, hipMemcpyHostToDevice, c->copy_stream) != hipSuccess ||
                    (nb_q && hipMemcpyAsync(c->ak_quals.p, quals + b->offsets[0], nb_q, hipMemcpyHostToDevice, c->copy_stream) != hipSuccess) ||
                    hipStreamSynchronize(c->copy_stream) != hipSuccess) rc_up = MONI_ENODEV;
            });
        }
        struct JoinGuard { std::thread& t; ~JoinGuard() { if (t.joinable()) t.join(); } } join_guard{uploader};
        static const bool use_fast = getenv("MONI_ALIGN_V1") == nullptr;
        moni_seed_params_t sp;
        sp.min_len = prm->min_len; sp.filter_seeds = prm->filter_seeds; sp.n_seeds_thr = prm->n_seeds_thr; sp.report_mems = 0;
        {
            const double t0 = mh::now_s();
            if (!resident && (rc = reads_upload(c, b, false))) return rc;
            if ((rc = seed_run_align(c, &sp))) return rc;
            st.t_seed += mh::now_s() - t0;
        }
        t_mark[0] = mh::now_s() - t_enter;
        const double t_gpu0 = mh::now_s();
        double t_launch[3] = {0, 0, 0};
        std::vector<int32_t> msc(c->max_len + 2);
        for (uint64_t l = 0; l <= c->max_len + 1; ++l) msc[l] = l ? (int32_t)(20 + 8 * log((double)l)) : INT32_MIN;
        const uint64_t cig_per = 16 * sub_reads + 4096, alt_per = 24 * sub_reads + 4096, md_per = 8 * sub_reads + 4096;
        const uint64_t txt_per = gpu_text ? 160 * sub_reads + 4096 : 0;
        if (uploader.joinable()) uploader.join();
        if (rc_up) return rc_up;
        if (gpu_text) {
            const uint32_t TAB = 8192;
            if ((rc = c->ak_txt.ensure(txt_per * n_sub + 8)) || (rc = c->h_txt.ensure(txt_per + 8)) || (rc = c->ak_mapq_tab.ensure(TAB))) return rc;
            if (!c->mapq_tab_ready) {
                std::vector<double> tab(TAB, 1.);
                const int32_t coeff_fac = (int32_t)log(50.0f);
                for (int32_t l = 2; l < (int32_t)TAB; ++l) tab[l] = coeff_fac / log(l);
                HIPCHK(hipMemcpy(c->ak_mapq_tab.p, tab.data(), TAB * sizeof(double), hipMemcpyHostToDevice));
                c->mapq_tab_ready = true;
            }
        }
        int n_cu = 256;
        n_cu = ctx_n_cu(c);
        const uint64_t ak_waves = use_fast ? std::min<uint64_t>(waves_full, 1024) : waves_full;
        if ((rc = c->ak_slots.ensure(AK_NSET * ak_waves * AK_NL)) || (rc = c->ak_waves.ensure(AK_NSET * ak_waves)) || (rc = c->h_recs.ensure(NR + 1)) ||
            (rc = c->h_cig.ensure(cig_per * n_sub + 1)) || (rc = c->h_alt.ensure(alt_per * n_sub + 1)) || (rc = c->h_md.ensure(md_per * n_sub + 1)) || (rc = c->ak_minscore.ensure(msc.size())) ||
            (rc = c->ak_cursors.ensure(AK_CUR * n_sub + AK_CUR)))
            return rc;
        const uint32_t af_slot_cap = (uint32_t)std::min<uint64_t>((uint64_t)AF_MAX_TASKS_READ * sub_reads + 4 * sub_reads + 4096, 0xFFFFFFF0ull);
        const uint32_t af_task_cap = (uint32_t)std::min<uint64_t>(12 * sub_reads + 4096, (1ull << AF_POS_BITS) - 1), af_tb_cap = (uint32_t)std::min<uint64_t>((4 + c->max_len / 50) * sub_reads + 1024, 0x7FFFFFFFull);
        const uint32_t af_chunk_cap = af_task_cap / 64 + 2 * AF_NBIN;
        uint64_t dirs_per_read = 16384;
        { const double f = (double)c->max_len / 150.0; if (f > 1.0) dirs_per_read = (uint64_t)(16384.0 * f * f); }
        dirs_per_read = std::min<uint64_t>(dirs_per_read * c->dirs_scale, 1ull << 20);
        const uint64_t af_dirs_cap = dirs_per_read * sub_reads + (16ull << 20);
        const unsigned af_dp_grid = (unsigned)n_cu * 12;
        const unsigned af_fin_grid = (unsigned)std::min<uint64_t>((sub_reads + 63) / 64, (uint64_t)n_cu * 16);
        const bool inorder = use_fast && gpu_text && ctx_out && force_back == 0 && getenv("MONI_ALIGN_HOST_ORDER") == nullptr;
        if (inorder && ((rc = c->ak_recs.ensure(NR + 1)) || (rc = c->ak_block.ensure(txt_per * n_sub + 8)) || (rc = c->ak_dev_len.ensure(NR + n_sub + 8)) || (rc = c->ak_dev_off.ensure(NR + n_sub + 8)) ||
                        (rc = c->ak_dev_pos.ensure(NR + 2 * n_sub + 8)) || (rc = c->ak_dev_sum.ensure(160 * n_sub + 8)) || (rc = c->h_sum.ensure(4 * n_sub + 4)))) return rc;
        size_t gather_tmp_bytes = 0;
        if (inorder) {
            if (rocprim::exclusive_scan(nullptr, gather_tmp_bytes, (uint64_t*)nullptr, (uint64_t*)nullptr, (uint64_t)0, (size_t)sub_reads, rocprim::plus<uint64_t>(), c->stream) != hipSuccess) return MONI_ENODEV;
            for (int x = 0; x < AK_NSET; ++x) if ((rc = c->gather_tmp[x].ensure(gather_tmp_bytes + 16))) return rc;
        }
        if (inorder) { HIPCHK(hipMemsetAsync(c->ak_dev_sum.p, 0, (160 * n_sub + 8) * sizeof(unsigned long long), c->stream)); memset(c->h_sum.p, 0, (4 * n_sub + 4) * sizeof(unsigned long long)); }
        if (use_fast) for (int x = 0; x < (int)std::min<uint64_t>(n_sub, AK_NSET); ++x) {
            moni_ctx::AfSet& S = c->af[x];
            if ((rc = S.plans.ensure(sub_reads + 1)) || (rc = S.tasks.ensure(af_slot_cap)) || (rc = S.res.ensure(af_slot_cap)) || (rc = S.ntasks.ensure(sub_reads + 8)) || (rc = S.bin_q.ensure((size_t)(AF_NBIN + 1) * af_task_cap)) ||
                (rc = S.task_pos.ensure(af_slot_cap)) || (rc = S.tb_task.ensure(af_tb_cap)) || (rc = S.tb.ensure(af_tb_cap)) || (rc = S.big_list.ensure(3 * (sub_reads + 1))) || (rc = S.ctab.ensure((size_t)(sub_reads + 1) * AF_CTAB)) ||
                (rc = S.ctr.ensure(AF_NCTR)) || (rc = S.txt_cur.ensure(AF_TXT_SHARDS * 8)) || (rc = S.bnd.ensure((size_t)af_dp_grid * AF_QCAP * 64)) || (rc = S.chunks.ensure(af_chunk_cap)) || (rc = S.dirs.ensure(af_dirs_cap)) || (rc = S.fin.ensure((size_t)af_fin_grid * 64 * sizeof(af_fin_t))) || (gpu_text && !fin_v1 && (rc = S.recipes.ensure((size_t)(sub_reads + 1) * AFP_WORDS))))
                return rc;
        }
        for (int x = 0; x < AK_NSET; ++x) if (!c->ak_stream[x]) HIPCHK(hipStreamCreateWithFlags(&c->ak_stream[x].h, hipStreamNonBlocking));
        if (!c->copy_stream) HIPCHK(hipStreamCreateWithFlags(&c->copy_stream.h, hipStreamNonBlocking));
        while (c->ak_done.size() < n_sub) { Event e0, e1, e2; HIPCHK(hipEventCreate(&e0.h)); HIPCHK(hipEventCreate(&e1.h)); HIPCHK(hipEventCreate(&e2.h));
                                            c->ak_begin.push_back(std::move(e0)); c->ak_done.push_back(std::move(e1)); c->ak_fin.push_back(std::move(e2)); }
        for (int x = 0; x < AK_NSET; ++x) if (use_fast && !c->fb_stream[x]) HIPCHK(hipStreamCreateWithFlags(&c->fb_stream[x].h, hipStreamNonBlocking));
        while (c->af_ev.size() < 3 * n_sub) { Event e; HIPCHK(hipEventCreate(&e.h)); c->af_ev.push_back(std::move(e)); }
        if (use_fast) { if ((rc = c->fb_all.ensure(16 * n_sub + n_sub * (sub_reads + 1) + 16))) return rc; HIPCHK(hipMemsetAsync(c->fb_all.p, 0, 16 * n_sub * sizeof(uint32_t), c->stream)); }
        HIPCHK(hipMemsetAsync(c->ak_cursors.p, 0, (AK_CUR * n_sub + AK_CUR) * sizeof(unsigned long long), c->stream));
        HIPCHK(hipMemcpyAsync(c->ak_minscore.p, msc.data(), msc.size() * 4, hipMemcpyHostToDevice, c->stream));
        HIPCHK(hipStreamSynchronize(c->stream));
        t_launch[0] = mh::now_s() - t_enter;
        if ((rc = c->af_ctr_host.ensure(AF_NCTR * n_sub + AF_NCTR))) return rc;
        memset(c->af_ctr_host.p, 0, AF_NCTR * n_sub * sizeof(uint32_t));
        struct SubRes { moni_aln_rec_t* recs = nullptr; uint32_t* cig = nullptr; moni_alt_t* alt = nullptr; const uint64_t* md = nullptr; const uint64_t* txt = nullptr; uint64_t nr = 0; };
        int rc_host = MONI_OK;
        auto fetch = [&](uint64_t k, SubRes& R) -> int {
            const uint64_t r0 = sub_lo[k], nr = sub_lo[k + 1] - sub_lo[k];
            const double f0 = mh::now_s();
            HIPCHK(hipEventSynchronize(c->ak_done[k]));
            const double f1 = mh::now_s();
            if (inorder && nr) { HIPCHK(hipMemcpyAsync(c->h_recs.p + r0, c->ak_recs.p + r0, nr * sizeof(moni_aln_rec_t), hipMemcpyDeviceToHost, c->copy_stream)); HIPCHK(hipStreamSynchronize(c->copy_stream)); }
            R.recs = c->h_recs.p + r0; R.cig = c->h_cig.p + k * cig_per; R.alt = c->h_alt.p + k * alt_per; R.md = c->h_md.p + k * md_per; R.nr = nr;
            if (getenv("MONI_AK_PROFILE")) fprintf(stderr, "  sub-batch %llu: waited for the launch from %.1f to %.1f ms\n", (unsigned long long)k, (f0 - t_enter) * 1e3, (f1 - t_enter) * 1e3);
            if (force_back) for (uint64_t r = 0; r < nr; ++r) if ((r0 + r) % force_back == 0) R.recs[r].status = 2;
            if (gpu_text) {
                const uint64_t n_reg = use_fast ? AF_TXT_SHARDS + 1 : 1, reg_words = use_fast ? txt_per / (AF_TXT_SHARDS + 1) : txt_per;
                uint64_t used[AF_TXT_SHARDS + 1];
                for (uint64_t g = 0; g < n_reg; ++g) used[g] = 0;
                for (uint64_t r = 0; r < nr; ++r) if (R.recs[r].txt_len) {
                    const uint64_t end = R.recs[r].txt_off + ((R.recs[r].txt_len + 7) >> 3);
                    const uint64_t g = R.recs[r].txt_off / reg_words;
                    if (g >= n_reg || end > (g + 1) * reg_words) return MONI_EINVAL;
                    used[g] = std::max(used[g], end - g * reg_words);
                }
                bool any = false;
                for (uint64_t g = 0; g < n_reg; ++g) if (used[g]) {
                    HIPCHK(hipMemcpyAsync(c->h_txt.p + g * reg_words, c->ak_txt.p + k * txt_per + g * reg_words, used[g] * 8, hipMemcpyDeviceToHost, c->copy_stream));
                    any = true;
                }
                if (any) HIPCHK(hipStreamSynchronize(c->copy_stream));
                R.txt = c->h_txt.p;
            }
            { float ms = 0; if (hipEventElapsedTime(&ms, c->ak_begin[k], c->ak_done[k]) == hipSuccess) { c->dp_kernel_ms_accum += ms; c->ak_kernel_ms = ms; } }
            return MONI_OK;
        };
        auto host_stage = [&](uint64_t k, const SubRes& R) {
            const double t0 = mh::now_s();
            const uint64_t r0 = sub_lo[k], nr = R.nr;
            for (uint64_t r = 0; r < nr; ++r) if (R.recs[r].status == 2) back_of[k].push_back((uint32_t)(r0 + r));
            bool oom = false;
            mh::parallel_for(pool, nr, [&](int t, size_t lo, size_t hi) {
                mh::Aligner::OutBuf& ob = c->pieces[t];
                static_assert(sizeof(moni_alt_t) == sizeof(mh::moni_alt_like), "alt record layout");
                std::vector<char>& mds = c->md_scratch[t];
                for (size_t r = lo; r < hi; ++r) {
                    const moni_aln_rec_t& Rr = R.recs[r];
                    if (Rr.status == 2) continue;
                    const uint64_t g = r0 + r;
                    const uint64_t off = b->offsets[g]; const uint32_t m = (uint32_t)(b->offsets[g + 1] - off);
                    if (R.txt && Rr.txt_len) {
                        if (!ob.ensure(Rr.txt_len)) { oom = true; break; }
                        memcpy(ob.base + ob.len, (const char*)(R.txt + Rr.txt_off), Rr.txt_len);
                        ob.len += Rr.txt_len;
                        if (Rr.status == 1) aligned_t[t]++;
                        continue;
                    }
                    if (!AL.emit_record(ob, mds, (const char*)names + name_off[g], (size_t)(name_off[g + 1] - name_off[g]), b->seq + off, quals ? quals + off : nullptr, m,
                                        Rr.status == 1, Rr.strand, Rr.ref_pos, Rr.score, Rr.score2, R.cig + Rr.cigar_off, Rr.n_cigar,
                                        (const mh::moni_alt_like*)R.alt + Rr.alt_off, Rr.n_alt,
                                        Rr.status == 1 ? (const char*)(R.md + Rr.md_off) : nullptr, Rr.md_len, Rr.nm, Rr.lift_nm)) { oom = true; break; }
                    if (Rr.status == 1) aligned_t[t]++;
                }
            });
            if (oom) eager_oom = true;
            if (eager_ok && back_of[k].empty() && !eager_oom) {
                std::vector<size_t> at(T + 1, alen);
                for (int t = 0; t < T; ++t) at[t + 1] = at[t] + c->pieces[t].len;
                const size_t need = at[T];
                if (need + 1 > acap) {
                    const size_t sub_bytes = need - alen, rest = NR - (r0 + nr);
// ... 38 lines not shown
                    host_busy += mh::now_s() - h0;
                    return;
                }
            }
            if ((rc_host = fetch(k, R))) return;
            if (k + 1 == n_sub) { t_mark[1] = mh::now_s() - t_enter; st.t_dp += mh::now_s() - t_gpu0; }
            host_stage(k, R);
        };
        uint64_t retired = 0, launched = 0;
        auto retire = [&](bool block) {
            while (retired < launched && !rc_host && !eager_oom) {
                if (!block && sub_lo[retired + 1] > sub_lo[retired] && hipEventQuery(c->ak_done[retired]) != hipSuccess) break;
                handle(retired);
                ++retired;
            }
        };
        for (uint64_t k = 0; k < n_sub; ++k) {
            const uint64_t r0 = sub_lo[k], nr = sub_lo[k + 1] - sub_lo[k];
            uint64_t n_waves = ak_waves;
            if (!use_fast && n_waves * AK_NL > nr) n_waves = (nr + AK_NL - 1) / AK_NL;
            waves_used = std::max(waves_used, n_waves);
            ak_args_t A;
            memset(&A, 0, sizeof A);
            A.P.min_len = prm->min_len; A.P.ext_len = prm->ext_len; A.P.check_k = prm->check_k; A.P.region_dist = prm->region_dist;
            A.P.filter_freq = prm->filter_freq; A.P.left_mem_check = prm->left_mem_check; A.P.freq_thr = prm->freq_thr;
            A.P.smatch = prm->smatch; A.P.gapo = prm->gapo; A.P.gapo2 = prm->gapo2; A.P.gape = prm->gape; A.P.gape2 = prm->gape2;
            A.P.max_dist_x = prm->max_dist_x; A.P.max_dist_y = prm->max_dist_y; A.P.max_iter = prm->max_iter; A.P.max_pred = prm->max_pred;
            A.P.min_chain_score = prm->min_chain_score; A.P.min_chain_length = prm->min_chain_length;
            A.P.n_text = I->K.n_text; A.P.n_seq = I->K.n_seq; A.P.seq_starts = I->d_seq_starts.p;
            A.P.lift_seqs = I->d_lift_seqs.p; A.P.lift_runs = I->d_lift_runs.p; A.P.pdir = I->d_pdir.p;
            A.D.sc_mch = prm->smatch; A.D.sc_mis = -prm->smismatch; A.D.sc_N = -prm->gape; A.D.wild = 4; A.D.qo = prm->gapo; A.D.e = prm->gape;
            A.D.end_bonus = prm->end_bonus; A.D.reads = c->seq.p; A.D.text = I->d_text.p; A.D.n_text = I->K.n_text;
            A.D.reads_limit = (c->total_len + 8) & ~7ull; A.D.text_limit = (I->K.n_text + 8) & ~7ull;
            A.mems = c->mems.p; A.occs = c->tmp.p; A.read_mem_off = c->read_mem_off.p; A.offs = c->offs.p;
            A.min_score_of_len = c->ak_minscore.p; A.max_len = (uint32_t)c->max_len + 1; A.read_lo = r0; A.n_reads = nr;
            A.slots = c->ak_slots.p + (k % AK_NSET) * ak_waves * AK_NL; A.waves = c->ak_waves.p + (k % AK_NSET) * ak_waves;
            A.recs = (inorder ? c->ak_recs.p : c->h_recs.p) + r0; A.cig_pool = c->h_cig.p + k * cig_per; A.cig_cap = cig_per; A.alt_pool = c->h_alt.p + k * alt_per;
            A.alt_cap = alt_per; A.md_pool = c->h_md.p + k * md_per; A.md_cap = md_per; A.cursors = c->ak_cursors.p + AK_CUR * k;
            if (gpu_text) {
                A.fmt.rnames = c->ak_rnames.p; A.fmt.rname_off = c->ak_rname_off.p; A.fmt.quals = quals ? c->ak_quals.p : nullptr;
                A.fmt.snames = I->d_snames.p; A.fmt.sname_off = I->d_sname_off.p; A.fmt.mapq_tab = c->ak_mapq_tab.p; A.fmt.mapq_tab_n = 8192;
                A.fmt.min_len = (int32_t)prm->min_len; A.fmt.smatch = prm->smatch; A.fmt.smismatch = prm->smismatch;
                A.fmt.txt_pool = c->ak_txt.p + k * txt_per; A.fmt.txt_cap = (use_fast && nr > 0) ? txt_per / (AF_TXT_SHARDS + 1) : txt_per;
            }
            if (inorder) { A.dev_len = c->ak_dev_len.p + r0 + k; A.dev_off = c->ak_dev_off.p + r0 + k; A.dev_sum = c->ak_dev_sum.p + 160 * k; }
            hipStream_t sx = c->ak_stream[k % AK_NSET];
            HIPCHK(hipEventRecord(c->ak_begin[k], sx));
            bool done_recorded = false;
            if (use_fast && nr > 0) {
                moni_ctx::AfSet& S = c->af[k % AK_NSET];
                af_args_t G;
                memset(&G, 0, sizeof G);
                G.A = A;
                G.plans = S.plans.p; G.tasks = S.tasks.p; G.task_cap = af_slot_cap; G.ntasks = S.ntasks.p; G.res = S.res.p; G.bin_q = S.bin_q.p; G.bin_cap = af_task_cap; G.task_pos = S.task_pos.p;
                G.chunks = S.chunks.p; G.chunk_cap = af_chunk_cap; G.dirs = S.dirs.p; G.dirs_cap = af_dirs_cap; G.tb_task = S.tb_task.p; G.tb = S.tb.p; G.tb_cap = af_tb_cap;
                G.fb_n = c->fb_all.p + 16 * k; G.fb_list = c->fb_all.p + 16 * n_sub + k * (sub_reads + 1); G.big_list = S.big_list.p; G.huge_list = S.big_list.p + (sub_reads + 1); G.list0 = S.big_list.p + 2 * (sub_reads + 1); G.fin_scratch = S.fin.p; G.fin_stride = sizeof(af_fin_t); G.ctr = S.ctr.p;
                G.bnd = S.bnd.p;
                G.pat = c->pat.p; G.blk = c->blk.p; G.text2 = I->d_text2.p; G.exc = I->d_exc.p; G.exc_sh = I->exc_sh; G.pflag = c->pflag.p; G.wave_max = af_wave_max();
                G.txt_cur = S.txt_cur.p; G.txt_shard_words = txt_per / (AF_TXT_SHARDS + 1);
                G.chain_narrow = cc_narrow_ok(A.P) ? 1u : 0u;
                HIPCHK(hipMemsetAsync(S.txt_cur.p, 0, AF_TXT_SHARDS * 8 * sizeof(unsigned long long), sx));
#ifdef AF_PROFILE
                if ((rc = S.prof.ensure(32))) return rc;
                if (k < AK_NSET) HIPCHK(hipMemsetAsync(S.prof.p, 0, 32 * 8, sx));
                G.prof = S.prof.p;
                if (const char* v = getenv("MONI_AF_DBG")) G.dbg = (uint32_t)atoi(v);
                {
                    const size_t pp_stride = (size_t)AFPP_WAVE * ((sub_reads + 63) / 64 + 1) + (size_t)AFPP_READ * (sub_reads + 1);
                    if ((rc = S.prep_prof.ensure(pp_stride * ((n_sub + AK_NSET - 1) / AK_NSET)))) return rc;
                    G.prep_prof = S.prep_prof.p + pp_stride * (k / AK_NSET);
                    HIPCHK(hipMemsetAsync(G.prep_prof, 0, pp_stride * sizeof(unsigned long long), sx));
                }
#endif
#ifdef AF_CUTS
                if (const char* v = getenv("MONI_AF_DBG")) G.dbg = (uint32_t)atoi(v);
#endif
                if (const char* v = getenv("MONI_AF_DBG")) G.dbg |= (uint32_t)atoi(v) & (64u | 65536u | 131072u);
                HIPCHK(hipMemsetAsync(S.ctr.p, 0, AF_NCTR * sizeof(uint32_t), sx));
                static const int l0_force = getenv("MONI_AF_L0") ? atoi(getenv("MONI_AF_L0")) : -1;
                const bool l0_mid = l0_force >= 0 ? l0_force == 1 : c->max_len > 200;
                G.l0_mm = l0_mid ? (uint32_t)af_wave_mid_t::MM : (uint32_t)af_wave_small_t::MM; G.l0_ma = l0_mid ? (uint32_t)af_wave_mid_t::MA : (uint32_t)af_wave_small_t::MA;
                const bool no_k2 = getenv("MONI_AF_NOPLANK") != nullptr;
                G.ctab = (no_k2 || l0_mid) ? nullptr : S.ctab.p;
                hipLaunchKernelGGL(classify_kernel, dim3((unsigned)((nr + 255) / 256)), dim3(256), 0, sx, G);
#define AF_LAUNCH_CP(WT, LEVEL, OCC, GW, grid) do { \
                    if ((G.dbg & 64) || !G.chain_narrow) hipLaunchKernelGGL((chain_plan_kernel<WT, LEVEL, OCC, GW, true>), grid, dim3(64), 0, sx, G); \
                    else hipLaunchKernelGGL((chain_plan_kernel<WT, LEVEL, OCC, GW, false>), grid, dim3(64), 0, sx, G); } while (0)
                if (l0_mid) {
                    const dim3 g1((unsigned)std::min<uint64_t>(nr, (uint64_t)n_cu * 4 * 4));
                    AF_LAUNCH_CP(af_wave_mid_t, 0, 4, 64, g1);
                } else {
                    static const int l0_gw = getenv("MONI_AF_GW") ? atoi(getenv("MONI_AF_GW")) : 64;
                    static const int k1occ = getenv("MONI_AF_K1OCC") ? atoi(getenv("MONI_AF_K1OCC")) : (l0_gw == 16 ? 2 : 8);
                    const dim3 g1((unsigned)std::min<uint64_t>(l0_gw == 16 ? (nr + 3) / 4 : nr, (uint64_t)n_cu * 4 * k1occ));
                    if (l0_gw == 16) AF_LAUNCH_CP(af_wave_small_t, 0, 2, 16, g1);
                    else if (k1occ == 4) AF_LAUNCH_CP(af_wave_small_t, 0, 4, 64, g1);
                    else if (k1occ == 5) AF_LAUNCH_CP(af_wave_small_t, 0, 5, 64, g1);
                    else if (k1occ == 8) AF_LAUNCH_CP(af_wave_small_t, 0, 8, 64, g1);
                    else AF_LAUNCH_CP(af_wave_small_t, 0, 6, 64, g1);
                }
                AF_LAUNCH_CP(af_wave_t, 1, 3, 64, dim3((unsigned)std::min<uint64_t>(nr, (uint64_t)n_cu * 10)));
                static const bool no_huge = getenv("MONI_AF_NOHUGE") != nullptr;
                if (!no_huge) AF_LAUNCH_CP(af_wave_huge_t, 2, 1, 64, dim3((unsigned)std::min<uint64_t>(nr, (uint64_t)n_cu)));
#undef AF_LAUNCH_CP
                HIPCHK(hipGetLastError());
                if (G.ctab) hipLaunchKernelGGL(plan_kernel, dim3((unsigned)((nr + 255) / 256)), dim3(256), 0, sx, G);
                hipLaunchKernelGGL(bin_tasks_kernel, dim3((unsigned)((nr + AF_BT_READS - 1) / AF_BT_READS)), dim3(256), 0, sx, G);
                HIPCHK(hipEventRecord(c->af_ev[3 * k], sx));
                af_launch_dp(G, sx, af_dp_grid, (unsigned)n_cu, nr);
                HIPCHK(hipEventRecord(c->af_ev[3 * k + 1], sx));
                hipLaunchKernelGGL(select_kernel, dim3((unsigned)((nr + 255) / 256)), dim3(256), 0, sx, G);
                hipLaunchKernelGGL(traceback_kernel, dim3((unsigned)((af_tb_cap + 255) / 256)), dim3(256), 0, sx, G);
                HIPCHK(hipEventRecord(c->af_ev[3 * k + 2], sx));
                A.read_list = G.fb_list; A.n_reads_dev = G.fb_n;
                hipStream_t sf = c->fb_stream[k % AK_NSET];
                HIPCHK(hipStreamWaitEvent(sf, c->af_ev[3 * k + 2], 0));
                hipLaunchKernelGGL(align_kernel, dim3((unsigned)ak_waves), dim3(64), 0, sf, A);
                static const int fin_mult = getenv("MONI_AF_FINGRID") ? atoi(getenv("MONI_AF_FINGRID")) : 96;
                if (gpu_text && !fin_v1) {
                    hipLaunchKernelGGL(finish_prep_kernel, dim3((unsigned)std::min<uint64_t>((nr + 63) / 64, (uint64_t)n_cu * 32)), dim3(64), 0, sx, G, S.recipes.p);
                    hipLaunchKernelGGL(finish_render_kernel, dim3((unsigned)std::min<uint64_t>(nr, (uint64_t)n_cu * fin_mult)), dim3(64), 0, sx, G, (const uint32_t*)S.recipes.p);
                } else if (gpu_text) hipLaunchKernelGGL(finish_wave_kernel, dim3((unsigned)std::min<uint64_t>(nr, (uint64_t)n_cu * fin_mult)), dim3(64), 0, sx, G);
                else hipLaunchKernelGGL(finish_kernel, dim3((unsigned)std::min<uint64_t>((nr + 63) / 64, af_fin_grid)), dim3(64), 0, sx, G);
                HIPCHK(hipMemcpyAsync(c->af_ctr_host.p + AF_NCTR * k, S.ctr.p, AF_NCTR * sizeof(uint32_t), hipMemcpyDeviceToHost, sx));
                HIPCHK(hipEventRecord(c->ak_fin[k], sx));
                HIPCHK(hipStreamWaitEvent(sf, c->ak_fin[k], 0));
                if (inorder) {
                    uint64_t* pos = c->ak_dev_pos.p + r0 + 2 * k;
                    size_t tmp_bytes = 0;
                    if (rocprim::exclusive_scan(nullptr, tmp_bytes, A.dev_len, pos, (uint64_t)0, nr, rocprim::plus<uint64_t>(), sf) != hipSuccess || tmp_bytes > gather_tmp_bytes + 16) return MONI_ENODEV;
                    if (rocprim::exclusive_scan(c->gather_tmp[k % AK_NSET].p, tmp_bytes, A.dev_len, pos, (uint64_t)0, nr, rocprim::plus<uint64_t>(), sf) != hipSuccess) return MONI_ENODEV;
                    hipLaunchKernelGGL(gather_lines_kernel, dim3((unsigned)std::min<uint64_t>((nr + 3) / 4, (uint64_t)n_cu * 8)), dim3(256), 0, sf, (const uint64_t*)A.fmt.txt_pool,
                                       (const uint64_t*)A.dev_len, (const uint64_t*)A.dev_off, (const uint64_t*)pos, nr, reinterpret_cast<uint8_t*>(c->ak_block.p + k * txt_per));
                    hipLaunchKernelGGL(gather_summary_kernel, dim3(1), dim3(64), 0, sf, (const uint64_t*)A.dev_len, (const uint64_t*)pos, nr, (const unsigned long long*)A.dev_sum,
                                       c->ak_dev_sum.p + 160 * k + 150);
                    HIPCHK(hipMemcpyAsync(c->h_sum.p + 4 * k, c->ak_dev_sum.p + 160 * k + 150, 3 * sizeof(unsigned long long), hipMemcpyDeviceToHost, sf));
                }
                HIPCHK(hipEventRecord(c->ak_done[k], sf));
                done_recorded = true;
            } else if (nr > 0) {
                hipLaunchKernelGGL(align_kernel, dim3((unsigned)n_waves), dim3(64), 0, sx, A);
            }
            if (!done_recorded) HIPCHK(hipEventRecord(c->ak_done[k], sx));
            HIPCHK(hipGetLastError());
            launched = k + 1;
        }
        t_launch[1] = mh::now_s() - t_enter;
        if (rc_host == MONI_OK) retire(true);
        if (rc_host) { for (int x = 0; x < AK_NSET; ++x) { (void)hipStreamSynchronize(c->ak_stream[x]); if (c->fb_stream[x]) (void)hipStreamSynchronize(c->fb_stream[x]); } drop_abuf(); return rc_host; }
        t_mark[2] = mh::now_s() - t_enter;
        st.dp_rounds = n_sub;
        bool any_dirs_ovf_batch = false;
        if (n_sub) {
            std::vector<unsigned long long> cur(AK_CUR * n_sub);
            HIPCHK(hipMemcpy(cur.data(), c->ak_cursors.p, cur.size() * sizeof(unsigned long long), hipMemcpyDeviceToHost));
            std::vector<uint32_t> fbn(16 * n_sub, 0);
            if (use_fast) HIPCHK(hipMemcpy(fbn.data(), c->fb_all.p, fbn.size() * sizeof(uint32_t), hipMemcpyDeviceToHost));
            for (uint64_t k = 0; k < n_sub; ++k) {
                const unsigned long long* q = cur.data() + AK_CUR * k;
                st.dp_tasks += q[2]; st.dp_cells += q[3]; st.dp_reused += q[8]; st.dp_cells_reused += q[9];
                if (use_fast && sub_lo[k + 1] > sub_lo[k]) {
                    float ms = 0;
                    if (hipEventElapsedTime(&ms, c->ak_begin[k], c->af_ev[3 * k]) == hipSuccess) st.t_k_chain += ms / 1e3;
                    if (hipEventElapsedTime(&ms, c->af_ev[3 * k], c->af_ev[3 * k + 1]) == hipSuccess) st.t_k_dp += ms / 1e3;
                    if (hipEventElapsedTime(&ms, c->af_ev[3 * k + 1], c->af_ev[3 * k + 2]) == hipSuccess) st.t_k_select += ms / 1e3;
                    if (hipEventElapsedTime(&ms, c->af_ev[3 * k + 2], c->ak_fin[k]) == hipSuccess) st.t_k_finish += ms / 1e3;
                }
                if (use_fast) {
                    const uint32_t* fc = c->af_ctr_host.p + AF_NCTR * k;
                    unsigned long long cells, rb, cutc, slots; memcpy(&cells, fc + AFC_CELLS, 8); memcpy(&rb, fc + AFC_RBYTES, 8); memcpy(&cutc, fc + AFC_CUTCELLS, 8); memcpy(&slots, fc + AFC_SLOTS, 8);
                    st.dp_cells_cut += cutc; st.dp_slots += slots;
                    any_dirs_ovf_batch = any_dirs_ovf_batch || fc[AFC_DIRS_OVF] != 0;
                    st.dp_tasks += fc[AFC_NT] + (fc[AFC_TASKS] >= (uint32_t)(sub_lo[k + 1] - sub_lo[k]) * AF_MAX_TASKS_READ ? fc[AFC_TASKS] - (uint32_t)(sub_lo[k + 1] - sub_lo[k]) * AF_MAX_TASKS_READ : 0u); st.dp_cells += cells; st.kernel_fallback += fbn[16 * k]; st.dp_ref_bytes += rb;
                    for (int x = 0; x < AF_WHY_N; ++x) why_sum[x] += fc[AFC_WHY + x];
                    if (getenv("MONI_AK_PROFILE")) { unsigned long long du; memcpy(&du, fc + AFC_DIROFF, 8); fprintf(stderr, "  direction bits of sub-batch %llu: %.1f MB used of %.1f MB\n", (unsigned long long)k, du / 1e6, af_dirs_cap / 1e6); }
                    if (getenv("MONI_AK_PROFILE")) fprintf(stderr, "  staged kernels, sub-batch %llu: %u DP tasks, %llu cells, %u traced, %u large + %u small + %u global chunks, %u reads to align_kernel%s\n",
                                                           (unsigned long long)k, fc[AFC_NT], cells, fc[AFC_TRACED], fc[AFC_NCHUNKS], fc[AFC_NCHUNKS + 1], fc[AFC_NCHUNKS + 2], fbn[16 * k], fc[AFC_DIRS_OVF] ? " (direction bytes overflowed)" : "");
                    if (getenv("MONI_AK_PROFILE")) { fprintf(stderr, "    DP problems per bin (16 of the large tile by query length <= 8 13 16 24 32 48 64 .. 160 192 224 256, 3 of the small tile <= 8 16 32, 16 global by query length / 16):"); for (int x = 0; x < AF_NBIN; ++x) fprintf(stderr, " %u", fc[AFC_BINS + x]); fprintf(stderr, "\n"); }
#if defined(AF_CUTS)
                    if (getenv("MONI_AK_PROFILE")) { fprintf(stderr, "    tile problems (extension | gap fill q = t | gap fill q != t) x (band <= 16 | wider | extension with t < q | no bound):"); for (int x = 0; x < 12; ++x) fprintf(stderr, "%s %u", x % 4 == 0 ? " |" : "", fc[180 + x]); fprintf(stderr, "\n"); }
#endif
                    if (getenv("MONI_AK_PROFILE")) { fprintf(stderr, "    global problems by band width / 4 (0-3, 4-7, ... , >= 52):"); for (int x = 0; x < 14; ++x) fprintf(stderr, " %u", fc[AFC_BANDH + x]); fprintf(stderr, "\n"); }
                    if (getenv("MONI_AK_PROFILE")) fprintf(stderr, "    handed over because: long read %u, anchors/seeds %u, chains %u, chains to score %u, chain length %u, DP size %u, overlapping anchors %u, wildcard %u, "
                                                           "loop depends on a score %u, extension short of the query end %u, capacity %u, CIGAR %u\n",
                                                           fc[AFC_WHY + 0], fc[AFC_WHY + 1], fc[AFC_WHY + 2], fc[AFC_WHY + 3], fc[AFC_WHY + 4], fc[AFC_WHY + 5], fc[AFC_WHY + 6], fc[AFC_WHY + 7], fc[AFC_WHY + 8], fc[AFC_WHY + 9], fc[AFC_WHY + 10], fc[AFC_WHY + 11]);
                }
                prof[0] += (double)q[5]; prof[1] += (double)q[6]; prof[2] += (double)q[7]; for (int x = 0; x < 4; ++x) prof[3 + x] += (double)q[10 + x];
                for (int x = 0; x < 8; ++x) hist[x] += (double)q[16 + x];
                for (int x = 0; x < 7; ++x) cyc[x] += (double)q[24 + x];
            }
        }
        if (any_dirs_ovf_batch && c->dirs_scale < 32) c->dirs_scale *= 2;
        static_assert(AF_WHY_N == 12, "moni_align_stats_t::handover_why");
        for (int x = 0; x < AF_WHY_N; ++x) why_out[x] = why_sum[x];
#ifdef AF_PROFILE
        if (use_fast && n_sub) { unsigned long long pf[32]; for (int x = 0; x < (int)std::min<uint64_t>(n_sub, AK_NSET); ++x) { HIPCHK(hipMemcpy(pf, c->af[x].prof.p, sizeof pf, hipMemcpyDeviceToHost));
            fprintf(stderr, "chain_plan_kernel wave cycles (set %d): load+filter+anchors %.3g, chain %.3g (sort %.3g, dp %.3g, ends+backtrack %.3g), lifts %.3g, plan %.3g, whole read %.3g\n", x,
                    (double)pf[0], (double)pf[1], (double)pf[5], (double)pf[6], (double)pf[7], (double)pf[2], (double)pf[3], (double)pf[4]);
            fprintf(stderr, "finish_wave_kernel wave cycles (set %d): stage + stitch + lift %.3g, MD / NM / MAPQ %.3g, segment list %.3g, render %.3g, out %.3g, whole read %.3g\n", x,
                    (double)pf[16], (double)pf[17], (double)pf[18], (double)pf[19], (double)pf[21], (double)pf[22]); } }
        if (use_fast && gpu_text && !fin_v1) for (uint64_t k = 0; k < n_sub; ++k) {
            const uint64_t nr = sub_lo[k + 1] - sub_lo[k];
            if (!nr) continue;
            const size_t pp_stride = (size_t)AFPP_WAVE * ((sub_reads + 63) / 64 + 1) + (size_t)AFPP_READ * (sub_reads + 1);
            const size_t nw = (size_t)std::min<uint64_t>((nr + 63) / 64, (uint64_t)n_cu * 32);
            std::vector<unsigned long long> pp(AFPP_WAVE * nw + AFPP_READ * nr);
            HIPCHK(hipMemcpy(pp.data(), c->af[k % AK_NSET].prep_prof.p + pp_stride * (k / AK_NSET), pp.size() * sizeof(unsigned long long), hipMemcpyDeviceToHost));
            unsigned long long first = ~0ull, last_start = 0, last_end = 0; size_t slow = 0; std::vector<unsigned long long> dur(nw);
            for (size_t w = 0; w < nw; ++w) {
                const unsigned long long* W = pp.data() + AFPP_WAVE * w;
                first = std::min(first, W[0]); last_start = std::max(last_start, W[0]); last_end = std::max(last_end, W[1]); dur[w] = W[1] - W[0];
                if (dur[w] > dur[slow]) slow = w;
            }
            std::vector<unsigned long long> sd(dur); std::sort(sd.begin(), sd.end());
            const unsigned long long* W = pp.data() + AFPP_WAVE * slow;
            fprintf(stderr, "finish_prep_kernel sub-batch %llu (%llu reads, %zu wavefronts): span %.3f ms, last wavefront starts at %.3f ms; wavefront time median %.3f ms, 99 %% %.3f ms, max %.3f ms\n",
                    (unsigned long long)k, (unsigned long long)nr, nw, (last_end - first) / 1e5, (last_start - first) / 1e5, sd[nw / 2] / 1e5, sd[nw * 99 / 100] / 1e5, sd[nw - 1] / 1e5);
            fprintf(stderr, "  slowest wavefront %zu (reads %llu..): starts at %.3f ms, ends at %.3f ms; cycles: stitch %llu, lift %llu, MAPQ + sequences %llu, MD %llu, MD of the unlifted %llu, alternatives %llu\n",
                    slow, (unsigned long long)(sub_lo[k] + 64 * slow), (W[0] - first) / 1e5, (W[1] - first) / 1e5, W[2], W[3], W[4], W[5], W[6], W[7]);
            if (sd[nw - 1] > 4 * sd[nw / 2]) {
                fprintf(stderr, "  its lanes (operations of the CIGAR / of the lifted one / MD items / alternatives / to the host; run hint, runs of the lift):");
                for (size_t l = 0; l < 64 && 64 * slow + l < nr; ++l) { const unsigned long long* R = pp.data() + AFPP_WAVE * nw + AFPP_READ * (64 * slow + l);
                    fprintf(stderr, " [%zu: %llu/%llu/%llu/%llu/%llu; %lld, %llu]", l, R[0] & 0xFFFF, (R[0] >> 16) & 0xFFFF, (R[0] >> 32) & 0xFFFF, (R[0] >> 48) & 0xFF, (R[0] >> 56) & 1, (long long)(int32_t)(uint32_t)R[1], R[1] >> 32); }
                fprintf(stderr, "\n");
            }
        }
#endif
        double ak_sum_ms = c->dp_kernel_ms_accum;
        if (n_sub) { float ms = 0; if (hipEventElapsedTime(&ms, c->ak_begin[0], c->ak_done[n_sub - 1]) == hipSuccess) c->dp_kernel_ms_accum = ms; }
        if (getenv("MONI_AK_PROFILE")) fprintf(stderr, "align_kernel: %.3f ms span (%.3f ms summed) in %llu launches, %llu waves x %d reads in flight; wave cycles: take+chain %.3g, later drives %.3g, DP %.3g; lane cycles in ac_init: load %.3g sort %.3g chain-dp %.3g backtrack %.3g\n", c->dp_kernel_ms_accum, ak_sum_ms, (unsigned long long)n_sub, (unsigned long long)waves_used, (int)AK_NL, prof[0], prof[1], prof[2], prof[3], prof[4], prof[5], prof[6]);
        if (getenv("MONI_AK_PROFILE")) fprintf(stderr, "DP problems run, by live rows min(qlen,tlen) <=16 / <=32 / <=64 / >64: count %.3g %.3g %.3g %.3g, cells %.3g %.3g %.3g %.3g\n",
                                               hist[0], hist[1], hist[2], hist[3], hist[4], hist[5], hist[6], hist[7]);
        if (getenv("MONI_AK_PROFILE")) fprintf(stderr, "wave cycles inside the DP phase: per-read setup %.3g, memo lookups %.3g, DP by live rows <=16 / <=32 / <=64 / >64: %.3g %.3g %.3g %.3g; 1x1 problems answered in closed form: %.3g\n",
                                               cyc[0], cyc[1], cyc[2], cyc[3], cyc[4], cyc[5], cyc[6]);
        st.dp_reused += (uint64_t)cyc[6];
        double t0 = mh::now_s();
        for (int t = 0; t < T; ++t) st.aligned += aligned_t[t];
        st.reads = NR;
        std::vector<uint32_t> back;
        for (auto& v : back_of) back.insert(back.end(), v.begin(), v.end());
        std::vector<std::string> back_line(back.size());
        if (!back.empty()) {
            std::vector<uint8_t> sseq, snames, squal; std::vector<uint64_t> soff(1, 0), snoff(1, 0);
            for (uint32_t r : back) {
                const uint64_t off = b->offsets[r], m = b->offsets[r + 1] - b->offsets[r];
                sseq.insert(sseq.end(), b->seq + off, b->seq + off + m); soff.push_back(sseq.size());
                snames.insert(snames.end(), names + name_off[r], names + name_off[r + 1]); snoff.push_back(snames.size());
                if (quals) squal.insert(squal.end(), quals + off, quals + off + m);
            }
            moni_read_batch_t sub{sseq.data(), soff.data(), (uint64_t)back.size()};
            std::string sout; mh::AlignStats s2;
            if ((rc = host_align_subset(c, *prm, sub, snames.data(), snoff.data(), quals ? squal.data() : nullptr, sout, s2))) { drop_abuf(); return rc; }
            size_t p0 = 0;
            for (size_t x = 0; x < back.size(); ++x) { const size_t p1 = sout.find('\n', p0); back_line[x] = sout.substr(p0, p1 - p0 + 1); p0 = p1 + 1; }
            st.aligned += s2.aligned; st.dp_tasks += s2.dp_tasks; st.dp_cells += s2.dp_cells; st.dp_rounds += s2.dp_rounds;
            st.t_chain += s2.t_chain;
        }
        st.handed_back = back.size();
        if (eager_oom) { drop_abuf(); return MONI_ENOMEM; }
        if (back.empty() && eager_upto == n_sub && (abuf || NR == 0)) {
            if (!abuf && !grow_abuf(64)) return MONI_ENOMEM;
            abuf[alen] = 0;
            *sam = abuf; *sam_len = alen;
            out_done = true;
        } else {
            if (abuf) { out.assign(abuf, alen); drop_abuf(); }
            size_t bi = 0;
            for (uint64_t k = eager_upto; k < n_sub; ++k) {
                const uint64_t r0 = sub_lo[k], nr = sub_lo[k + 1] - sub_lo[k];
                for (int t = 0; t < T; ++t) {
                    const size_t lo = (nr < 2 || T <= 1) ? (t == 0 ? 0 : nr) : nr * t / T, hi = (nr < 2 || T <= 1) ? (t == 0 ? nr : nr) : nr * (t + 1) / T;
                    const std::string& piece = kept[k][t];
                    size_t p0 = 0;
                    for (size_t r = lo; r < hi; ++r) {
                        if (bi < back.size() && back[bi] == r0 + r) { out += back_line[bi++]; continue; }
                        const size_t p1 = piece.find('\n', p0);
                        out.append(piece, p0, p1 - p0 + 1); p0 = p1 + 1;
                    }
                }
            }
        }
        st.t_host += host_busy + (mh::now_s() - t0);
        if (getenv("MONI_AK_PROFILE")) fprintf(stderr, "align_core wall: launches queued from %.1f to %.1f ms\n", t_launch[0] * 1e3, t_launch[1] * 1e3);
        if (getenv("MONI_AK_PROFILE")) fprintf(stderr, "align_core wall: seeded at %.1f ms, last launch done at %.1f, last host stage done at %.1f, text ready at %.1f\n",
                                               t_mark[0] * 1e3, t_mark[1] * 1e3, t_mark[2] * 1e3, (mh::now_s() - t_enter) * 1e3);
    }
    if (!out_done) {
        char* dst;
        if (ctx_out) {
            if (c->out_buf.ensure_keep(out.size() + 1, 0)) return MONI_ENOMEM;
            dst = c->out_buf.p;
        } else if (!(dst = (char*)malloc(out.size() + 1))) return MONI_ENOMEM;
        memcpy(dst, out.data(), out.size());
        dst[out.size()] = 0;
        *sam = dst; *sam_len = out.size();
    }
    if (stats) {
        stats->reads = st.reads; stats->aligned = st.aligned; stats->dp_tasks = st.dp_tasks; stats->dp_cells = st.dp_cells; stats->dp_rounds = st.dp_rounds;
        stats->t_seed = st.t_seed; stats->t_chain = st.t_chain; stats->t_dp = st.t_dp; stats->t_host = st.t_host;
        stats->t_dp_kernel = c->dp_kernel_ms_accum / 1e3;
        stats->handed_back = st.handed_back; stats->dp_reused = st.dp_reused; stats->dp_cells_reused = st.dp_cells_reused;
        stats->kernel_fallback = st.kernel_fallback; stats->dp_ref_bytes = st.dp_ref_bytes; stats->dp_cells_cut = st.dp_cells_cut; stats->dp_slots = st.dp_slots;
        stats->t_k_chain = st.t_k_chain; stats->t_k_dp = st.t_k_dp; stats->t_k_select = st.t_k_select; stats->t_k_finish = st.t_k_finish;
        for (int x = 0; x < 12; ++x) stats->handover_why[x] = why_out[x];
    }
    return MONI_OK;
}

int moni_report_mems_batch(moni_ctx_t* c, const moni_read_batch_t* b, const uint8_t* names, const uint64_t* name_off, const uint8_t* quals,
                           const moni_align_params_t* prm, char** sam, uint64_t* sam_len) {
    if (!c || !b || !prm || !sam || !sam_len || (b->n_reads && (!names || !name_off))) return MONI_EINVAL;
    int rc = moni_reads_upload(c, b);
    if (rc) return rc;
    moni_seed_params_t sp;
    sp.min_len = prm->min_len; sp.filter_seeds = prm->filter_seeds; sp.n_seeds_thr = prm->n_seeds_thr; sp.report_mems = 1;
    if ((rc = seed_run_align(c, &sp))) return rc;
    try {
        std::vector<moni_mem_t> mems(c->n_mems); std::vector<uint64_t> occs(c->n_occs), rmo(c->n_reads + 1);
        if ((rc = moni_seed_fetch(c, mems.data(), occs.data(), rmo.data()))) return rc;
        const mh::HostIndex& ix = c->idx->hix;
        std::string out;
        char num[32];
        for (uint64_t r = 0; r < c->n_reads; ++r) {
            const uint64_t off = b->offsets[r], m = b->offsets[r + 1] - off;
            size_t total = 0;
            for (uint64_t k = rmo[r]; k < rmo[r + 1]; ++k) total += mems[k].occ_cnt;
            for (uint64_t k = rmo[r]; k < rmo[r + 1]; ++k) {
                const moni_mem_t& M = mems[k];
                if (prm->filter_freq) { const double fr = static_cast<double>(M.occ_cnt) / total; if (fr > prm->freq_thr) continue; }
                const bool rc_strand = (M.mate & 2) != 0;
                std::string seq(M.len, 'N'), ql;
                for (uint32_t x = 0; x < M.len; ++x) seq[x] = rc_strand ? (char)mh::compl_of(b->seq[off + m - 1 - (M.idx + x)]) : (char)b->seq[off + M.idx + x];
                if (quals) { ql.resize(M.len); for (uint32_t x = 0; x < M.len; ++x) ql[x] = rc_strand ? (char)quals[off + m - 1 - (M.idx + x)] : (char)quals[off + M.idx + x]; }
                for (uint32_t j = 0; j < M.occ_cnt; ++j) {
                    const auto ref = ix.index(occs[M.occ_off + j]);
                    out.append((const char*)names + name_off[r], (size_t)(name_off[r + 1] - name_off[r]));
                    out += rc_strand ? "\t272\t" : "\t256\t";
                    out += ix.names[ref.first]; out.push_back('\t');
                    snprintf(num, sizeof num, "%d", (int)(ref.second + 1)); out += num;
                    out += "\t255\t"; snprintf(num, sizeof num, "%d", (int)M.len); out += num; out += "M\t*\t0\t0\t";
                    out += seq; out.push_back('\t');
                    if (quals) out += ql; else out.push_back('*');
                    out += "\tAS:i:0\tNM:i:0\tMD:Z:\tOA:Z:*,0,"; out += rc_strand ? "-" : "+"; out += ",*,255,0;\tAA:Z:\n";
                }
            }
        }
        char* dst = (char*)malloc(out.size() + 1);
        if (!dst) return MONI_ENOMEM;
        memcpy(dst, out.data(), out.size()); dst[out.size()] = 0;
        *sam = dst; *sam_len = out.size();
        return MONI_OK;
    } catch (const std::bad_alloc&) { return MONI_ENOMEM; }
}

__global__ void lift_batch_kernel(const ac_params_t P, const uint64_t* __restrict__ pos, uint64_t n, uint64_t* __restrict__ out) {
    const uint64_t i = (uint64_t)blockIdx.x * blockDim.x + threadIdx.x;
    if (i < n) out[i] = ac_lift(P, pos[i]);
}

int moni_ms_file_info(const char* path, uint64_t* n, uint64_t* r) {
    if (!path) return MONI_EINVAL;
    try {
        uint64_t a = 0, b = 0;
        int rc = msio::info_ms(path, a, b);
        if (rc) return rc;
        if (n) *n = a;
        if (r) *r = b;
        return MONI_OK;
    } catch (const std::bad_alloc&) { return MONI_ENOMEM; }
}

int moni_ms_file_read(const char* path, uint64_t r, uint64_t* F, uint8_t* heads, uint64_t* starts, uint64_t* ssa, uint64_t* esa, uint64_t* thr, uint64_t* slcp,
                      char* err, uint64_t err_cap) {
    if (!path || !F || !heads || !starts || !ssa || !esa || !thr || !slcp) return MONI_EINVAL;
    try {
        msio::MsFile M; std::string e;
        int rc = msio::load_ms(path, M, e);
        if (rc) { if (err && err_cap) snprintf(err, (size_t)err_cap, "%s", e.c_str()); return rc; }
        if (M.r != r) return MONI_EINVAL;
        memcpy(F, M.F.data(), 256 * 8); memcpy(heads, M.heads.data(), r); memcpy(starts, M.starts.data(), (r + 1) * 8);
        memcpy(ssa, M.ssa.data(), r * 8); memcpy(esa, M.esa.data(), r * 8); memcpy(thr, M.thr.data(), r * 8); memcpy(slcp, M.slcp.data(), r * 8);
        return MONI_OK;
    } catch (const std::bad_alloc&) { return MONI_ENOMEM; }
}

int moni_ms_file_write(const moni_flat_index_t* f, const char* path) {
    if (!f || !path || !f->F || !f->heads || !f->starts || !f->ssa || !f->esa || !f->thr || f->r < 1 || f->n < 2) return MONI_EINVAL;
// ... 131 lines not shown
```

Measured before the change: 43.09 million.

## Route short-run reads from chain_plan to a per-run parallel chaining kernel

In the small-instance chain planner, reads whose anchor runs all hold at most 8 anchors (and no more than 16 runs) are staged to a global buffer and returned early. A new chain_runs_kernel then chains each run on its own lane, 16 lanes per read, using shared-memory columns. It ranks and sorts the kept chains and writes the anchor and chain tables directly, so the wave-serial chaining DP is no longer run for these reads. Reads that produce too many chains or anchors go to the big list instead. This costs an extra kernel launch, a memset, staging memory traffic, and more chaining paths to keep correct.

```diff
diff --git a/include/moni_hip.h b/include/moni_hip.h
--- a/include/moni_hip.h
+++ b/include/moni_hip.h
@@ -152,6 +152,7 @@
     uint64_t handover_why[12];
     uint64_t dp_cells_cut;
     uint64_t dp_slots;
+    uint64_t runs_routed;
 } moni_align_stats_t;
 
 void moni_align_params_default(moni_align_params_t *p);
diff --git a/moni_align_amd/capi.py b/moni_align_amd/capi.py
--- a/moni_align_amd/capi.py
+++ b/moni_align_amd/capi.py
@@ -69,7 +69,7 @@
                 ("t_dp_kernel", C.c_double), ("handed_back", C.c_uint64), ("dp_reused", C.c_uint64), ("dp_cells_reused", C.c_uint64),
                 ("kernel_fallback", C.c_uint64), ("dp_ref_bytes", C.c_uint64),
                 ("t_k_chain", C.c_double), ("t_k_dp", C.c_double), ("t_k_select", C.c_double), ("t_k_finish", C.c_double),
-                ("handover_why", C.c_uint64 * 12), ("dp_cells_cut", C.c_uint64), ("dp_slots", C.c_uint64)]
+                ("handover_why", C.c_uint64 * 12), ("dp_cells_cut", C.c_uint64), ("dp_slots", C.c_uint64), ("runs_routed", C.c_uint64)]
 
 
 class PeParamsC(C.Structure):
diff --git a/moni_align_amd/csrc/align_fast.hip b/moni_align_amd/csrc/align_fast.hip
--- a/moni_align_amd/csrc/align_fast.hip
+++ b/moni_align_amd/csrc/align_fast.hip
@@ -40,7 +40,8 @@
 #define AF_NEG_INF (-0x40000000)
 
 enum { AF_GAP_NONE = 0, AF_GAP_INS, AF_GAP_DEL0, AF_GAP_TASK, AF_GAP_1X1 };
-enum { AF_ST_UNALIGNED = 0, AF_ST_CAND = 1, AF_ST_FALLBACK = 2, AF_ST_FINAL = 3, AF_ST_CHAINS = 4  };
+enum { AF_ST_UNALIGNED = 0, AF_ST_CAND = 1, AF_ST_FALLBACK = 2, AF_ST_FINAL = 3, AF_ST_CHAINS = 4 ,
+       AF_ST_RUNS = 5  };
 
 struct af_anchor_t {
     uint64_t occ;
@@ -90,6 +91,12 @@
 struct af_ctab_t { int32_t score; uint16_t an0; uint8_t cnt, strand; uint64_t left_ref; };
 static_assert(sizeof(af_ctab_t) == 16, "af_ctab_t");
 #define AF_CTAB 48
+#define AF_RUN_LEN 8
+#define AF_RUN_SLOTS 16
+#define AF_RUN_CHAINS 48
+#define AF_RUN_NODES 96
+struct af_rstage_t { uint64_t node[AF_RUN_NODES]; uint64_t xbase[AF_RUN_SLOTS]; float avg; uint8_t na, n_runs, rs[AF_RUN_SLOTS + 1] , pad; };
+static_assert(sizeof(af_rstage_t) == 920 && AF_MAX_READ <= 1024 && AF_RUN_LEN <= 16 && AF_RUN_NODES <= 127 && AF_RUN_CHAINS <= 255, "af_rstage_t: field widths");
 struct af_res_t { int32_t mqe, mqe_t, score, flags; };
 struct af_chunk_t { uint32_t bin, start, n, qhi; uint64_t dir_off; };
 struct af_tb_t { uint32_t n_ops; uint32_t ops[AF_TB_CIG]; };
@@ -113,6 +120,7 @@
     const uint64_t* text2; const uint32_t* exc; uint32_t exc_sh;
     const uint8_t* pflag;
     af_ctab_t* ctab;
+    af_rstage_t* rstage; uint8_t* rflag;
     uint32_t* list0; uint32_t* big_list; uint32_t* huge_list;
     unsigned long long* txt_cur;
     uint64_t txt_shard_words;
@@ -144,6 +152,7 @@
        AFC_SLOTS = 48 ,
        AFC_CUTCELLS = 50 ,
        AFC_BANDH = 52 ,
+       AFC_RUNS = 66 ,
        AFC_BINS = 68 , AFC_WMODE = 172 , AF_NCTR = 192 };
 static_assert(AFC_BINS + AF_NBIN + 1 <= AFC_WMODE && AFC_WMODE + 7 <= AF_NCTR && AFC_WHY + 12 <= AFC_RBYTES && AFC_BANDH + 14 <= AFC_BINS && AFC_NCHUNKS + 7 <= AFC_CURSOR && AFC_CURSOR + 7 <= AFC_BIG, "counter layout");
 enum { AF_GRP_LARGE = 0, AF_GRP_SMALL = 1, AF_GRP_BAND = 2, AF_GRP_WILD = 3, AF_GRP_GLOBAL = 4, AF_GRP_GBAND = 5, AF_GRP_GWILD = 6 };
@@ -405,8 +414,8 @@
     }
 }
 
-template <class WT, class GT = af_grp_t<64>, bool GEN = true>
-__device__ __forceinline__ uint32_t af_chain(const af_args_t& G, WT& L, uint32_t na, float avg_mem_length, const GT g = GT(), const bool sec_on = false) {
+template <class WT, class GT = af_grp_t<64>, bool GEN = true, bool ROUTE = false>
+__device__ __forceinline__ uint32_t af_chain(const af_args_t& G, WT& L, uint32_t na, float avg_mem_length, const GT g = GT(), const bool sec_on = false, const uint32_t r_in = 0) {
     const ac_params_t& P = G.A.P;
     constexpr uint32_t GW = GT::W;
     const int lane = g.lane;
@@ -434,6 +443,23 @@
     }
     if (lane == 0) L.run_start[n_runs] = (uint16_t)na;
     __syncthreads();
+    if (ROUTE && G.rstage != nullptr && n_runs <= AF_RUN_SLOTS) {
+        const bool lng = (uint32_t)lane < n_runs && (uint32_t)L.run_start[lane + 1] - (uint32_t)L.run_start[lane] > AF_RUN_LEN;
+        if (g.ballot(lng) == 0) {
+            af_rstage_t& R = G.rstage[r_in];
+            for (uint32_t i = lane; i < na; i += GW) {
+                const uint64_t aw = L.anch[i];
+                const af_mem_t mi = L.mem[aw >> 40];
+                uint32_t fb = 0;
+                for (uint32_t k = 1; k < n_runs; ++k) { const uint32_t s = L.run_start[k]; fb = s <= i ? s : fb; }
+                R.node[i] = (AF_X(aw) - AF_X(L.anch[fb])) | ((uint64_t)mi.rpos << 32) | ((uint64_t)mi.len << 42) | ((uint64_t)mi.idx << 52) | ((uint64_t)mi.mate << 62);
+            }
+            if ((uint32_t)lane < n_runs) R.xbase[lane] = AF_X(L.anch[L.run_start[lane]]);
+            if ((uint32_t)lane <= n_runs) R.rs[lane] = (uint8_t)L.run_start[lane];
+            if (lane == 0) { R.avg = avg_mem_length; R.na = (uint8_t)na; R.n_runs = (uint8_t)n_runs; G.rflag[r_in] = (uint8_t)n_runs; }
+            return AF_ST_RUNS;
+        }
+    }
 #if defined(AF_PROFILE) || defined(AF_CUTS)
     if (G.dbg & 128) return AF_ST_UNALIGNED;
 #endif
@@ -794,10 +820,12 @@
 #if defined(AF_PROFILE) || defined(AF_CUTS)
     if (G.dbg & 4) na = 0;
 #endif
+    constexpr bool ROUTE = LEVEL == 0 && !GEN && GW == 64 && !WT::SEC && (uint32_t)WT::MA <= AF_RUN_NODES && (uint32_t)WT::MC <= AF_CTAB && (uint32_t)WT::MA <= AF_PLAN_AN;
     if (!fallback && !too_big && na > 0) {
-        status = af_chain<WT, GT, GEN>(G, L, na, avg, g);
+        status = af_chain<WT, GT, GEN, ROUTE>(G, L, na, avg, g, false, r_in);
         status = (uint32_t)g.shfl((int)status, 0);
         __syncthreads();
+        if (ROUTE && status == AF_ST_RUNS) return;
 #if defined(AF_PROFILE) || defined(AF_CUTS)
         if ((G.dbg & 8) && status == AF_ST_CAND) status = AF_ST_UNALIGNED;
 #endif
@@ -963,6 +991,145 @@
         __syncthreads();
         af_plan_read<WT, LEVEL, GEN>(G, L, g, r_in, off, m, na, avg, fallback, too_big);
     }
+}
+
+struct af_runcol_t {
+    uint64_t (*node)[64]; int16_t (*fa)[64]; int16_t (*ma)[64]; int8_t (*pa)[64]; uint8_t (*ta)[64]; uint8_t (*sa)[64]; int lane;
+    __device__ __forceinline__ long long x(uint32_t k) const { return (long long)(uint32_t)node[k][lane]; }
+    __device__ __forceinline__ int32_t y(uint32_t k) const { return (int32_t)((node[k][lane] >> 32) & 1023u); }
+    __device__ __forceinline__ int32_t w(uint32_t k) const { return (int32_t)((node[k][lane] >> 42) & 1023u); }
+    __device__ __forceinline__ uint32_t mate(uint32_t k) const { return (uint32_t)(node[k][lane] >> 62); }
+    __device__ __forceinline__ int32_t f(uint32_t k) const { return fa[k][lane]; }
+    __device__ __forceinline__ int32_t msc(uint32_t k) const { return ma[k][lane]; }
+    __device__ __forceinline__ int32_t p(uint32_t k) const { return pa[k][lane]; }
+    __device__ __forceinline__ int32_t t(uint32_t k) const { return ta[k][lane]; }
+    __device__ __forceinline__ void set_f(uint32_t k, int32_t v) { fa[k][lane] = (int16_t)v; }
+    __device__ __forceinline__ void set_msc(uint32_t k, int32_t v) { ma[k][lane] = (int16_t)v; }
+    __device__ __forceinline__ void set_p(uint32_t k, int32_t v) { pa[k][lane] = (int8_t)v; }
+    __device__ __forceinline__ void set_t(uint32_t k, int32_t v) { ta[k][lane] = (uint8_t)v; }
+    __device__ __forceinline__ uint32_t start(uint32_t q) const { return sa[q][lane]; }
+    __device__ __forceinline__ void set_start(uint32_t q, uint32_t v) { sa[q][lane] = (uint8_t)v; }
+};
+static_assert(AF_RUN_NODES == af_wave_small_t::MA && AF_RUN_CHAINS == af_wave_small_t::MC && AF_RUN_CHAINS <= AF_CTAB && AF_RUN_NODES <= AF_PLAN_AN, "chain_runs_kernel holds what the small instance holds");
+__global__ void __launch_bounds__(64) chain_runs_kernel(const af_args_t G) {
+    __shared__ uint64_t s_node[AF_RUN_LEN][64];
+    __shared__ int16_t s_f[AF_RUN_LEN][64], s_msc[AF_RUN_LEN][64];
+    __shared__ int8_t s_p[AF_RUN_LEN][64];
+    __shared__ uint8_t s_t[AF_RUN_LEN][64], s_sj[AF_RUN_LEN][64];
+    __shared__ uint32_t s_key[4][AF_RUN_CHAINS], s_ord[4][AF_RUN_CHAINS], s_piece[4][AF_RUN_CHAINS];
+    __shared__ uint16_t s_ipos[4][AF_RUN_CHAINS], s_jpos[4][AF_RUN_CHAINS];
+    __shared__ lsort::frame s_stack[4][16];
+    __shared__ uint8_t s_cnt[4][AF_RUN_CHAINS];
+    const af_grp_t<16> g;
+    const int lane = threadIdx.x, grp = lane >> 4, slot = lane & 15;
+    const ak_args_t& A = G.A;
+    const ac_params_t& P = A.P;
+    const uint32_t n_work = G.ctr[AFC_L0];
+    af_runcol_t C{s_node, s_f, s_msc, s_p, s_t, s_sj, lane};
+    uint32_t n_routed = 0;
+    for (uint32_t w0 = blockIdx.x * 4u; w0 < n_work; w0 += gridDim.x * 4u) {
+        const uint32_t w = w0 + (uint32_t)grp;
+        const uint32_t r_in = w < n_work ? G.list0[w] : 0u;
+        const af_rstage_t& R = G.rstage[r_in];
+        const uint32_t n_runs = w < n_work ? G.rflag[r_in] : 0u;
+        const bool mine = (uint32_t)slot < n_runs;
+        uint32_t fb = 0, n = 0;
+        float avg = 0.f;
+        uint64_t xbase = 0;
+        if (mine) { fb = R.rs[slot]; n = (uint32_t)R.rs[slot + 1] - fb; avg = R.avg; xbase = R.xbase[slot]; }
+        if (n > AF_RUN_LEN) n = AF_RUN_LEN;
+        {
+            uint64_t v[AF_RUN_LEN];
+#pragma unroll
+            for (uint32_t q = 0; q < AF_RUN_LEN; ++q) v[q] = q < n ? R.node[fb + q] : 0ull;
+#pragma unroll
+            for (uint32_t q = 0; q < AF_RUN_LEN; ++q) { s_node[q][lane] = v[q]; s_t[q][lane] = 0; }
+        }
+        cc_run_dp<int32_t, uint32_t>(C, fb, n, (int32_t)P.max_iter, (uint32_t)P.max_pred, (long long)P.max_dist_x, (int32_t)P.max_dist_y, avg);
+        uint32_t ns = 0;
+        cc_run_starts(C, fb, n, P.min_chain_score, [&](uint32_t j) { C.set_start(ns++, j); });
+        uint32_t nk = 0, n_an = 0;
+        cc_run_chains(C, fb, n, ns, P.min_chain_score, P.min_chain_length, [](uint32_t) {},
+                      [&](uint32_t j0, int32_t, uint32_t cnt, bool keep) { if (keep) { s_msc[nk++][lane] = (int16_t)(j0 | (cnt << 8)); n_an += cnt; } });
+        uint32_t ns_all = ns, an_all = n_an, incl = nk;
+        for (int o = 1; o < 16; o <<= 1) { ns_all += (uint32_t)__shfl_xor((int)ns_all, o); an_all += (uint32_t)__shfl_xor((int)an_all, o); }
+        for (int o = 1; o < 16; o <<= 1) { const uint32_t up = (uint32_t)__shfl_up((int)incl, o, 16); if (slot >= o) incl += up; }
+        const uint32_t nk_all = (uint32_t)__shfl((int)incl, 15, 16);
+        const bool routed = n_runs > 0;
+        const bool big = routed && (ns_all > AF_RUN_CHAINS || an_all > AF_PLAN_AN);
+        const bool go = routed && !big;
+        if (go) for (uint32_t c = 0; c < nk; ++c) {
+            const uint32_t e = (uint32_t)(uint16_t)s_msc[c][lane], j = e & 0xFFu;
+            s_key[grp][incl - nk + c] = ((uint32_t)s_f[j - fb][lane] << 8) | j;
+            s_piece[grp][incl - nk + c] = e >> 8;
+        }
+        __syncthreads();
+#pragma unroll
+        for (uint32_t q = 0; q < (AF_RUN_CHAINS + 15) / 16; ++q) {
+            const uint32_t sidx = (uint32_t)slot + 16u * q;
+            if (go && sidx < nk_all) {
+                const uint32_t pos = cc_chain_pos(s_key[grp], nk_all, sidx);
+                s_ord[grp][pos] = (s_key[grp][sidx] & ~0xFFu) | pos;
+                s_cnt[grp][pos] = (uint8_t)s_piece[grp][sidx];
+                s_jpos[grp][sidx] = (uint16_t)pos;
+            }
+        }
+        __syncthreads();
+        if (go) for (uint32_t c = 0; c < nk; ++c) s_sj[c][lane] = (uint8_t)s_jpos[grp][incl - nk + c];
+        __syncthreads();
+        if (go && nk_all > 16) af_wave_sort<(AF_RUN_CHAINS + 15) / 16>(g, s_ord[grp], nk_all, s_stack[grp], s_ipos[grp], s_jpos[grp], s_piece[grp], [](const uint32_t& x) { return -(int32_t)(x >> 8); });
+        __syncthreads();
+        {
+            uint32_t an_base = 0;
+#pragma unroll
+            for (uint32_t q = 0; q < (AF_RUN_CHAINS + 15) / 16; ++q) {
+                const uint32_t k = (uint32_t)slot + 16u * q;
+                const bool in = go && k < nk_all;
+                const uint32_t o = in ? (s_ord[grp][k] & 0xFFu) : 0u;
+                const uint32_t cn = in ? (uint32_t)s_cnt[grp][o] : 0u;
+                uint32_t inc = cn;
+                for (int d = 1; d < 16; d <<= 1) { const uint32_t up = (uint32_t)__shfl_up((int)inc, d, 16); if (slot >= d) inc += up; }
+                if (in) { s_ipos[grp][o] = (uint16_t)k; s_jpos[grp][k] = (uint16_t)(an_base + inc - cn); }
+                an_base += (uint32_t)__shfl((int)inc, 15, 16);
+            }
+        }
+        __syncthreads();
+        if (go) {
+            af_ctab_t* const CT = G.ctab + (size_t)r_in * AF_CTAB;
+            af_anchor_t* const AN = G.plans[r_in].an;
+            for (uint32_t c = 0; c < nk; ++c) {
+                const uint32_t e = (uint32_t)(uint16_t)s_msc[c][lane], cnt = e >> 8;
+                const uint32_t rank = s_ipos[grp][s_sj[c][lane]], an0 = s_jpos[grp][rank];
+                int32_t j = (int32_t)(e & 0xFFu);
+                af_anchor_t X;
+                uint32_t mate = 0;
+                for (uint32_t q = 0; q < cnt; ++q) {
+                    const uint64_t nd = s_node[(uint32_t)j - fb][lane];
+                    const uint32_t len = (uint32_t)(nd >> 42) & 1023u;
+                    X.occ = xbase + (uint32_t)nd - len + 1; X.len = (uint16_t)len; X.idx = (uint16_t)((nd >> 52) & 1023u); X.gap_val = 0; X.gap_kind = AF_GAP_NONE; X.pad = 0;
+                    AN[an0 + cnt - 1 - q] = X;
+                    mate = (uint32_t)(nd >> 62);
+                    j = s_p[(uint32_t)j - fb][lane];
+                }
+                af_ctab_t E; E.score = (int32_t)(s_ord[grp][rank] >> 8); E.an0 = (uint16_t)an0; E.cnt = (uint8_t)cnt; E.strand = (mate & 2u) ? 1 : 0;
+                E.left_ref = ac_seq_off(P, ac_lift(P, X.occ)) + 1;
+                CT[rank] = E;
+            }
+            if (slot == 0) {
+                const uint64_t r = A.read_lo + r_in;
+                const uint32_t m = (uint32_t)(A.offs[r + 1] - A.offs[r]);
+                af_plan_t& PH = G.plans[r_in];
+                PH.status = ns_all == 0 ? AF_ST_UNALIGNED : AF_ST_CHAINS; PH.n_cand = 0; PH.n_chains = (uint16_t)nk_all; PH.final_cand = 0; PH.n_alt = 0; PH.pad = 0; PH.score2 = 0;
+                PH.ref_pos = PH.ref_len = 0; PH.tb0 = 0; PH.pad2 = 0;
+                PH.min_score = A.min_score_of_len[m <= A.max_len ? m : A.max_len];
+                G.ntasks[r_in] = 0;
+                ++n_routed;
+            }
+        } else if (big && slot == 0) G.big_list[atomicAdd(&G.ctr[AFC_BIG], 1u)] = r_in;
+        __syncthreads();
+    }
+    for (int o = 32; o > 0; o >>= 1) n_routed += (uint32_t)__shfl_xor((int)n_routed, o);
+    if (lane == 0 && n_routed) atomicAdd(&G.ctr[AFC_RUNS], n_routed);
 }
 
 struct af_plan_view_t { af_anchor_t* an; moni_dp_task_t* tasks; };
@@ -3068,6 +3235,7 @@
     }
 }
 
+static inline bool af_runs_on() { const char* v = getenv("MONI_AF_RUNS"); return !(v && atoi(v) == 0); }
 static inline uint32_t af_wave_max() { const char* v = getenv("MONI_AF_WAVE_MAX"); return v ? (uint32_t)strtoul(v, nullptr, 10) : 96u; }
 static inline void af_launch_dp(const af_args_t& G, hipStream_t sx, unsigned dp_grid, unsigned n_cu, uint64_t n_units) {
     if (!(G.dbg & 0x20000u)) hipLaunchKernelGGL(band_tasks_kernel, dim3((unsigned)((G.bin_cap + 255) / 256)), dim3(256), 0, sx, G);
diff --git a/moni_align_amd/csrc/chain_core.h b/moni_align_amd/csrc/chain_core.h
--- a/moni_align_amd/csrc/chain_core.h
+++ b/moni_align_amd/csrc/chain_core.h
@@ -43,3 +43,91 @@
     gain = alpha - beta;
     return true;
 }
+
+
+template <class I, class U, class S>
+CC_HD void cc_run_dp(S& s, uint32_t fb, uint32_t n, I max_iter, U max_pred, long long max_dist_x, I max_dist_y, float avg_mem_length) {
+    I lb = (I)fb;
+    for (uint32_t i = fb; i < fb + n; ++i) {
+        const uint32_t ki = i - fb;
+        const long long x_i = s.x(ki);
+        const I y_i = (I)s.y(ki), w_i = (I)s.w(ki);
+        const uint32_t mate_i = s.mate(ki);
+        I max_f = w_i, max_j = -1;
+        U n_pred = 0;
+        if ((U)i - (U)lb > (U)max_iter) lb = (I)i - max_iter;
+        for (I j = (I)i - 1; j >= lb; --j) {
+            const uint32_t kj = (uint32_t)j - fb;
+            const long long x_j = s.x(kj);
+            const uint32_t mate_j = s.mate(kj);
+            if (mate_i != mate_j && ((mate_i ^ mate_j) != 3)) continue;
+            if (x_i > x_j + max_dist_x) { lb = j; continue; }
+            I gain;
+            if (!cc_gain<I>((I)(x_i - x_j), y_i, (I)s.y(kj), w_i, mate_i == mate_j, max_dist_y, avg_mem_length, gain)) continue;
+            const I score = (I)s.f(kj) + gain;
+            if (score > max_f) { max_f = score; max_j = j; if (n_pred > 0) --n_pred; }
+            else if ((U)(I)s.t(kj) == (U)i && (++n_pred > max_pred)) break;
+            const I pj = (I)s.p(kj);
+            if (pj > 0) s.set_t((uint32_t)pj - fb, (I)i);
+        }
+        s.set_f(ki, max_f); s.set_p(ki, max_j);
+        I m = max_f;
+        if (max_j >= 0) { const I mp = (I)s.msc((uint32_t)max_j - fb); if (mp > max_f) m = mp; }
+        s.set_msc(ki, m);
+    }
+}
+
+template <class S, class Emit>
+CC_HD uint32_t cc_run_starts(S& s, uint32_t fb, uint32_t n, long long min_chain_score, Emit emit) {
+    for (uint32_t k = 0; k < n; ++k) s.set_t(k, 0);
+    for (uint32_t k = 0; k < n; ++k) { const int pk = (int)s.p(k); if (pk >= 0) s.set_t((uint32_t)pk - fb, 1); }
+    uint32_t ns = 0;
+    for (uint32_t k = 0; k < n; ++k) {
+        if (s.t(k) != 0 || !((long long)s.msc(k) > min_chain_score)) continue;
+        uint32_t j = k;
+        while (s.f(j) < s.msc(j)) j = (uint32_t)s.p(j) - fb;
+        emit(fb + j);
+        ++ns;
+    }
+    return ns;
+}
+
+CC_HD bool cc_start_before(long long fa, uint32_t ja, long long fb, uint32_t jb) { return fa > fb || (fa == fb && ja > jb); }
+
+template <class S, class Visit>
+CC_HD uint32_t cc_run_backtrack(S& s, uint32_t fb, uint32_t j0, long long min_chain_score, long long min_chain_length, bool& keep, Visit visit) {
+    const long long f0 = (long long)s.f(j0 - fb);
+    int j = (int)j0;
+    uint32_t cnt = 0;
+    do { visit((uint32_t)j); ++cnt; s.set_t((uint32_t)j - fb, 1); j = (int)s.p((uint32_t)j - fb); } while (j >= 0 && s.t((uint32_t)j - fb) == 0);
+    keep = false;
+    if (j < 0) keep = (long long)cnt >= min_chain_length;
+    else if (f0 - (long long)s.f((uint32_t)j - fb) >= min_chain_score) keep = (long long)cnt >= min_chain_length;
+    return cnt;
+}
+
+template <class S, class Visit, class Chain>
+CC_HD void cc_run_chains(S& s, uint32_t fb, uint32_t n, uint32_t ns, long long min_chain_score, long long min_chain_length, Visit visit, Chain chain) {
+    for (uint32_t k = 0; k < n; ++k) s.set_t(k, 0);
+    for (uint32_t it = 0; it < ns; ++it) {
+        uint32_t best = 0xFFu, bj = 0; int32_t bf = 0;
+        for (uint32_t q = 0; q < ns; ++q) {
+            const uint32_t j = (uint32_t)s.start(q);
+            if (j == 0xFFu) continue;
+            const int32_t fj = (int32_t)s.f(j - fb);
+            if (best == 0xFFu || cc_start_before(fj, j, bf, bj)) { best = q; bj = j; bf = fj; }
+        }
+        s.set_start(best, 0xFF);
+        bool keep;
+        const uint32_t cnt = cc_run_backtrack(s, fb, bj, min_chain_score, min_chain_length, keep, visit);
+        chain(bj, bf, cnt, keep);
+    }
+}
+
+CC_HD uint32_t cc_chain_pos(const uint32_t* key, uint32_t n, uint32_t c) {
+    const uint32_t kc = key[c];
+    uint32_t pos = 0;
+#pragma unroll 8
+    for (uint32_t s = 0; s < n; ++s) pos += (key[s] > kc || (key[s] == kc && s < c)) ? 1u : 0u;
+    return pos;
+}
diff --git a/moni_align_amd/csrc/moni_hip.hip b/moni_align_amd/csrc/moni_hip.hip
--- a/moni_align_amd/csrc/moni_hip.hip
+++ b/moni_align_amd/csrc/moni_hip.hip
@@ -162,7 +162,7 @@
     DBuf<uint8_t> dp_dir_big;
     struct AfSet {
         DBuf<af_plan_t> plans; DBuf<moni_dp_task_t> tasks; DBuf<af_res_t> res; DBuf<uint32_t> bin_q, task_pos, tb_task, big_list, ctr; DBuf<uint8_t> ntasks;
-        DBuf<af_chunk_t> chunks; DBuf<uint8_t> dirs, fin; DBuf<uint32_t> recipes; DBuf<af_ctab_t> ctab; DBuf<af_tb_t> tb; DBuf<uint64_t> bnd; DBuf<unsigned long long> prof, prep_prof, txt_cur;
+        DBuf<af_chunk_t> chunks; DBuf<uint8_t> dirs, fin; DBuf<uint32_t> recipes; DBuf<af_ctab_t> ctab; DBuf<af_rstage_t> rstage; DBuf<uint8_t> rflag; DBuf<af_tb_t> tb; DBuf<uint64_t> bnd; DBuf<unsigned long long> prof, prep_prof, txt_cur;
     } af[AK_NSET], af_pe[PE_NSET];
     HBuf<unsigned long long> pe_hcur;
     HBuf<uint32_t> af_ctr_host;
@@ -1163,6 +1163,7 @@
     std::string out;
     mh::AlignStats st;
     uint64_t why_out[12] = {};
+    uint64_t runs_routed = 0;
     const uint8_t* q = quals ? quals + b->offsets[0] : nullptr;
     static const bool host_only = getenv("MONI_ALIGN_HOST") != nullptr;
     bool out_done = false;
@@ -1293,7 +1294,7 @@
         if (use_fast) for (int x = 0; x < (int)std::min<uint64_t>(n_sub, AK_NSET); ++x) {
             moni_ctx::AfSet& S = c->af[x];
             if ((rc = S.plans.ensure(sub_reads + 1)) || (rc = S.tasks.ensure(af_slot_cap)) || (rc = S.res.ensure(af_slot_cap)) || (rc = S.ntasks.ensure(sub_reads + 8)) || (rc = S.bin_q.ensure((size_t)(AF_NBIN + 1) * af_task_cap)) ||
-                (rc = S.task_pos.ensure(af_slot_cap)) || (rc = S.tb_task.ensure(af_tb_cap)) || (rc = S.tb.ensure(af_tb_cap)) || (rc = S.big_list.ensure(3 * (sub_reads + 1))) || (rc = S.ctab.ensure((size_t)(sub_reads + 1) * AF_CTAB)) ||
+                (rc = S.task_pos.ensure(af_slot_cap)) || (rc = S.tb_task.ensure(af_tb_cap)) || (rc = S.tb.ensure(af_tb_cap)) || (rc = S.big_list.ensure(3 * (sub_reads + 1))) || (rc = S.ctab.ensure((size_t)(sub_reads + 1) * AF_CTAB)) || (af_runs_on() && ((rc = S.rstage.ensure(sub_reads + 1)) || (rc = S.rflag.ensure(sub_reads + 8)))) ||
                 (rc = S.ctr.ensure(AF_NCTR)) || (rc = S.txt_cur.ensure(AF_TXT_SHARDS * 8)) || (rc = S.bnd.ensure((size_t)af_dp_grid * AF_QCAP * 64)) || (rc = S.chunks.ensure(af_chunk_cap)) || (rc = S.dirs.ensure(af_dirs_cap)) || (rc = S.fin.ensure((size_t)af_fin_grid * 64 * sizeof(af_fin_t))) || (gpu_text && !fin_v1 && (rc = S.recipes.ensure((size_t)(sub_reads + 1) * AFP_WORDS))))
                 return rc;
         }
@@ -1498,6 +1499,13 @@
                 G.l0_mm = l0_mid ? (uint32_t)af_wave_mid_t::MM : (uint32_t)af_wave_small_t::MM; G.l0_ma = l0_mid ? (uint32_t)af_wave_mid_t::MA : (uint32_t)af_wave_small_t::MA;
                 const bool no_k2 = getenv("MONI_AF_NOPLANK") != nullptr;
                 G.ctab = (no_k2 || l0_mid) ? nullptr : S.ctab.p;
+                static const int l0_gw = getenv("MONI_AF_GW") ? atoi(getenv("MONI_AF_GW")) : 64;
+                G.rstage = (G.ctab && af_runs_on() && !(G.dbg & 64) && G.chain_narrow && l0_gw != 16) ? S.rstage.p : nullptr;
+#if defined(AF_PROFILE) || defined(AF_CUTS)
+                if (G.dbg & (4u | 8u | 16u | 32u | 128u | 256u | 512u | 1024u)) G.rstage = nullptr;
+#endif
+                G.rflag = S.rflag.p;
+                if (G.rstage) HIPCHK(hipMemsetAsync(S.rflag.p, 0, nr, sx));
                 hipLaunchKernelGGL(classify_kernel, dim3((unsigned)((nr + 255) / 256)), dim3(256), 0, sx, G);
 #define AF_LAUNCH_CP(WT, LEVEL, OCC, GW, grid) do { \
                     if ((G.dbg & 64) || !G.chain_narrow) hipLaunchKernelGGL((chain_plan_kernel<WT, LEVEL, OCC, GW, true>), grid, dim3(64), 0, sx, G); \
@@ -1506,7 +1514,6 @@
                     const dim3 g1((unsigned)std::min<uint64_t>(nr, (uint64_t)n_cu * 4 * 4));
                     AF_LAUNCH_CP(af_wave_mid_t, 0, 4, 64, g1);
                 } else {
-                    static const int l0_gw = getenv("MONI_AF_GW") ? atoi(getenv("MONI_AF_GW")) : 64;
                     static const int k1occ = getenv("MONI_AF_K1OCC") ? atoi(getenv("MONI_AF_K1OCC")) : (l0_gw == 16 ? 2 : 8);
                     const dim3 g1((unsigned)std::min<uint64_t>(l0_gw == 16 ? (nr + 3) / 4 : nr, (uint64_t)n_cu * 4 * k1occ));
                     if (l0_gw == 16) AF_LAUNCH_CP(af_wave_small_t, 0, 2, 16, g1);
@@ -1515,6 +1522,7 @@
                     else if (k1occ == 8) AF_LAUNCH_CP(af_wave_small_t, 0, 8, 64, g1);
                     else AF_LAUNCH_CP(af_wave_small_t, 0, 6, 64, g1);
                 }
+                if (G.rstage) hipLaunchKernelGGL(chain_runs_kernel, dim3((unsigned)std::min<uint64_t>((nr + 3) / 4, (uint64_t)n_cu * 40)), dim3(64), 0, sx, G);
                 AF_LAUNCH_CP(af_wave_t, 1, 3, 64, dim3((unsigned)std::min<uint64_t>(nr, (uint64_t)n_cu * 10)));
                 static const bool no_huge = getenv("MONI_AF_NOHUGE") != nullptr;
                 if (!no_huge) AF_LAUNCH_CP(af_wave_huge_t, 2, 1, 64, dim3((unsigned)std::min<uint64_t>(nr, (uint64_t)n_cu)));
@@ -1589,9 +1597,10 @@
                     any_dirs_ovf_batch = any_dirs_ovf_batch || fc[AFC_DIRS_OVF] != 0;
                     st.dp_tasks += fc[AFC_NT] + (fc[AFC_TASKS] >= (uint32_t)(sub_lo[k + 1] - sub_lo[k]) * AF_MAX_TASKS_READ ? fc[AFC_TASKS] - (uint32_t)(sub_lo[k + 1] - sub_lo[k]) * AF_MAX_TASKS_READ : 0u); st.dp_cells += cells; st.kernel_fallback += fbn[16 * k]; st.dp_ref_bytes += rb;
                     for (int x = 0; x < AF_WHY_N; ++x) why_sum[x] += fc[AFC_WHY + x];
+                    runs_routed += fc[AFC_RUNS];
                     if (getenv("MONI_AK_PROFILE")) { unsigned long long du; memcpy(&du, fc + AFC_DIROFF, 8); fprintf(stderr, "  direction bits of sub-batch %llu: %.1f MB used of %.1f MB\n", (unsigned long long)k, du / 1e6, af_dirs_cap / 1e6); }
-                    if (getenv("MONI_AK_PROFILE")) fprintf(stderr, "  staged kernels, sub-batch %llu: %u DP tasks, %llu cells, %u traced, %u large + %u small + %u global chunks, %u reads to align_kernel%s\n",
-                                                           (unsigned long long)k, fc[AFC_NT], cells, fc[AFC_TRACED], fc[AFC_NCHUNKS], fc[AFC_NCHUNKS + 1], fc[AFC_NCHUNKS + 2], fbn[16 * k], fc[AFC_DIRS_OVF] ? " (direction bytes overflowed)" : "");
+                    if (getenv("MONI_AK_PROFILE")) fprintf(stderr, "  staged kernels, sub-batch %llu: %u DP tasks, %llu cells, %u traced, %u large + %u small + %u global chunks, %u reads to align_kernel%s; %u of the small instance's %u reads chained by chain_runs_kernel\n",
+                                                           (unsigned long long)k, fc[AFC_NT], cells, fc[AFC_TRACED], fc[AFC_NCHUNKS], fc[AFC_NCHUNKS + 1], fc[AFC_NCHUNKS + 2], fbn[16 * k], fc[AFC_DIRS_OVF] ? " (direction bytes overflowed)" : "", fc[AFC_RUNS], fc[AFC_L0]);
                     if (getenv("MONI_AK_PROFILE")) { fprintf(stderr, "    DP problems per bin (16 of the large tile by query length <= 8 13 16 24 32 48 64 .. 160 192 224 256, 3 of the small tile <= 8 16 32, 16 global by query length / 16):"); for (int x = 0; x < AF_NBIN; ++x) fprintf(stderr, " %u", fc[AFC_BINS + x]); fprintf(stderr, "\n"); }
 #if defined(AF_CUTS)
                     if (getenv("MONI_AK_PROFILE")) { fprintf(stderr, "    tile problems (extension | gap fill q = t | gap fill q != t) x (band <= 16 | wider | extension with t < q | no bound):"); for (int x = 0; x < 12; ++x) fprintf(stderr, "%s %u", x % 4 == 0 ? " |" : "", fc[180 + x]); fprintf(stderr, "\n"); }
@@ -1719,6 +1728,7 @@
         stats->kernel_fallback = st.kernel_fallback; stats->dp_ref_bytes = st.dp_ref_bytes; stats->dp_cells_cut = st.dp_cells_cut; stats->dp_slots = st.dp_slots;
         stats->t_k_chain = st.t_k_chain; stats->t_k_dp = st.t_k_dp; stats->t_k_select = st.t_k_select; stats->t_k_finish = st.t_k_finish;
         for (int x = 0; x < 12; ++x) stats->handover_why[x] = why_out[x];
+        stats->runs_routed = runs_routed;
     }
     return MONI_OK;
 }
diff --git a/profiles/chain_runs_hist.py b/profiles/chain_runs_hist.py
--- /dev/null
+++ b/profiles/chain_runs_hist.py
@@ -0,0 +1,33 @@
+import os, sys, tempfile
+sys.path.insert(0, os.path.dirname(os.path.dirname(os.path.abspath(__file__))))
+import numpy as np
+from tests import chain_runs_model as T
+from moni_align_amd import index_build, synth
+from oracle import orc
+
+haps = int(sys.argv[1]) if len(sys.argv) > 1 else 12
+n = int(sys.argv[2]) if len(sys.argv) > 2 else 3000
+pg = synth.make_pangenome(200000, haps, seed=19, var_seed=12)
+fi = index_build.build_from_pangenome(pg, device="cpu")
+d = tempfile.mkdtemp(); p = os.path.join(d, "c.mfi"); fi.save(p)
+o = orc.OracleIndex(p)
+reads = synth.make_reads(pg, n, 150, seed=150)
+offs = np.arange(0, (n + 1) * 150, 150, dtype=np.uint64)
+w = o.seed_batch(reads.reshape(-1), offs, 25, True, 1000, threads=8)
+mems = np.zeros(len(w["pos"]), dtype=[(f, np.uint64) for f in ("pos", "len", "idx", "mate", "rpos", "occ_cnt", "occ_off")])
+for f in mems.dtype.names:
+    mems[f] = w[f]
+ms = T.models(dict(mems=mems, occs=w["occs"], read_mem_off=w["read_mem_off"]))
+def hist(key):
+    v = np.array([m[key] for m in ms]); return {int(k): int(c) for k, c in zip(*np.unique(v, return_counts=True))}
+print("sequences", len(pg.seqs), "reads", n)
+print("anchors/read mean", np.mean([m["n"] for m in ms]))
+print("runs per read", hist("n_runs"))
+print("longest run", hist("max_run"))
+rl = np.array([x for m in ms for x in m["run_lens"]]); print("anchors per run", {int(k): int(c) for k, c in zip(*np.unique(rl, return_counts=True))}, "mean %.2f" % rl.mean())
+print("kept chains", hist("kept"))
+print("starts", hist("starts"))
+l0 = [m for m in ms if m["n"] <= 96 and m["seeds"] <= 24]
+print("list0", len(l0), "gate", sum(m["gate"] for m in ms), "routed", sum(m["routed"] for m in ms))
+for rl in (4, 5, 6, 7, 8, 10, 12, 16):
+    print(" RUN_LEN", rl, "covers of list0:", sum(1 for m in l0 if m["n"] > 0 and m["max_run"] <= rl and m["n_runs"] <= 16) / max(1, len(l0)))
```

Measured after the change: 44.33 million (median of 6 runs). 1.03x the previous value.
